# FelipeMartins96/rsoccer-isaac-cleanrl

Hardware: AMD Instinct MI355X
Metric: env-steps/s (num_envs×horizon) at 65 536 envs; PPO wall-clock to 1e8 steps (higher is better)
Workload: dtype f32; 1 GPU; vss_step FULL contract: 65536 fields/GPU, one launch per control step, random actions (BASELINE configs[1]/[2] shape); fields_per_gpu=65536, mode=full, agent_rows_per_field=1, launch=eager ctypes launches, parallelism=fields sharded over 1 GPU(s), no data-path collective

## Files before the change

### include/vss.h

```cpp
#ifndef VSS_AMD_VSS_H
#define VSS_AMD_VSS_H

#include <stdint.h>

#ifdef __cplusplus
extern "C" {
#endif

#define VSS_ABI_VERSION 2

#define VSS_NUM_TEAMS 2
#define VSS_NUM_ROBOTS 3
#define VSS_NUM_AGENTS 6
#define VSS_NUM_OBS 52
#define VSS_NUM_ACTIONS 2
#define VSS_NUM_REW 4

#define VSS_CH_BALL_X 0
#define VSS_CH_BALL_Y 1
#define VSS_CH_BALL_VX 2
#define VSS_CH_BALL_VY 3
#define VSS_CH_RX 4
#define VSS_CH_RY 10
#define VSS_CH_RQX 16
#define VSS_CH_RQY 22
#define VSS_CH_RQZ 28
#define VSS_CH_RQW 34
#define VSS_CH_RVX 40
#define VSS_CH_RVY 46
#define VSS_CH_RW 52
#define VSS_STATE_CHANNELS 58

#define VSS_MODE_FULL 0
#define VSS_MODE_SA 1
#define VSS_MODE_CMA 2
#define VSS_MODE_DMA 3


#define VSS_OK 0
#define VSS_E_ARG 1
#define VSS_E_LAUNCH 2

typedef struct vss_params {
  float w_goal;
  float w_grad;
  float w_move;
  float w_energy;
  float clip_actions;
  int32_t max_episode_length;
  uint64_t seed;
} vss_params;

typedef struct vss_state {
  float* state;
  int64_t* progress_buf;
  int64_t* reset_buf;
  float* dof_velocity_buf;
  uint32_t* rng_counter;
} vss_state;

typedef struct vss_step_io {
  const float* actions;
  float* ou_buf;
  float* obs;
  float* terminal_obs;
  float* rew;
  float* reward_sum;
  int64_t* dones_rep;
  uint8_t* time_outs;
  float* progress_f;
} vss_step_io;

typedef struct vss_rollout_io {
  const float* actions;
  float* obs;
  float* terminal_obs;
  float* rew;
  int64_t* dones;
  uint8_t* time_outs;
  float* progress_f;
} vss_rollout_io;

typedef struct vss_replay_draws {
  const float* uniforms;
  int64_t uniform_stride;
  const float* normals;
} vss_replay_draws;

int vss_abi_version(void);

const char* vss_source_hash(void);

const char* vss_error_string(int code);

int vss_step(void* stream, int64_t n_fields, int32_t mode, const vss_params* params,
             const vss_state* st, const vss_step_io* io);

int vss_step_replay(void* stream, int64_t n_fields, int32_t mode, const vss_params* params,
                    const vss_state* st, const vss_step_io* io, const vss_replay_draws* draws);

typedef struct vss_versus_io {
  const float* opp_actions;
  float* opp_obs;
} vss_versus_io;

int vss_step_versus(void* stream, int64_t n_fields, int32_t mode, const vss_params* params,
                    const vss_state* st, const vss_step_io* io, const vss_versus_io* vs);

int vss_rollout(void* stream, int64_t n_fields, int32_t n_steps, const vss_params* params,
                const vss_state* st, const vss_rollout_io* io);

int vss_reset_dones(void* stream, int64_t n_fields, const vss_params* params,
                    const vss_state* st);

int vss_reset_dones_replay(void* stream, int64_t n_fields, const vss_params* params,
                           const vss_state* st, const vss_replay_draws* draws);

int vss_compute_observations(void* stream, int64_t n_fields, const vss_state* st,
                             float* obs, int32_t n_agents);


int64_t vss_mlp_packed_size(int32_t n_out);

int vss_mlp_pack(void* stream, int32_t n_out, const float* const* weights, const float* const* biases,
                 float* packed);

int vss_policy_forward(void* stream, int64_t rows, int32_t n_act, const float* obs,
                       const float* actor_packed, const float* logstd, const float* critic_packed,
                       uint64_t seed, uint64_t counter, const float* action_in, float* action_out,
                       float* logprob_out, float* entropy_out, float* value_out, float* mean_out);

int vss_value_forward_masked(void* stream, int64_t rows, int32_t n_act, const float* obs,
                             const float* actor_packed, const float* logstd, const float* critic_packed,
                             uint64_t seed, uint64_t counter, const float* action_in, float* action_out,
                             float* logprob_out, float* entropy_out, float* value_out, float* mean_out,
                             const int64_t* row_mask);

int vss_actor_forward(void* stream, int64_t rows, int32_t n_act, const float* obs, const float* actor_packed,
                      const float* logstd, uint64_t seed, uint64_t counter, float* action_out, float* mean_out);

int vss_policy_sample(void* stream, int64_t rows, int32_t n_act, const float* mean, const float* logstd, uint64_t seed,
                      uint64_t counter, const float* action_in, float* action_out, float* logprob_out,
                      float* entropy_out);

#define VSS_MAX_ACTOR_GROUPS 16
typedef struct vss_actor_groups {
  int32_t count;
  int64_t group_rows;
  const float* actor_packed[VSS_MAX_ACTOR_GROUPS];
  const float* logstd[VSS_MAX_ACTOR_GROUPS];
} vss_actor_groups;

int vss_actor_forward_grouped(void* stream, int64_t rows, int32_t n_act, const float* obs, const vss_actor_groups* g,
                              uint64_t seed, uint64_t counter, float* action_out, float* mean_out);

int vss_policy_sample_grouped(void* stream, int64_t rows, int32_t n_act, const float* mean, const vss_actor_groups* g,
                              uint64_t seed, uint64_t counter, float* action_out);

int64_t vss_tanh_grad_chunks(int64_t rows, int32_t cols);
int vss_tanh_grad_bias(void* stream, int64_t rows, int32_t cols, const float* grad_out, const float* y,
                       float* grad_in, float* bias_partial);

int vss_linear_tanh(void* stream, int64_t rows, int32_t k_in, int32_t n_out, const float* x, const float* w,
                    const float* bias, float* y);

int vss_linear_tanh_out(void* stream, int64_t rows, int32_t k_in, int32_t n_out, const float* x, const float* w,
                        const float* bias, float* y, int32_t k_out, const float* w_out, float* out_part);

int64_t vss_linear_tanh_backward_chunks(int64_t rows, int32_t k_next, int32_t n_out);
int vss_linear_tanh_backward(void* stream, int64_t rows, int32_t k_next, int32_t n_out, const float* grad_next,
                             const float* w_next_t, const float* y, float* grad_in, float* bias_partial);

int64_t vss_output_backward_chunks(int64_t rows, int32_t k_pad, int32_t n);
int vss_output_backward(void* stream, int64_t rows, int32_t k_pad, int32_t n, const float* g_out, const float* w_out_t,
                        const float* y, float* grad_in, float* bias_partial, float* wgrad_partial);

int64_t vss_output_backward_direct_chunks(int64_t rows, int32_t k_out, int32_t n);
int vss_output_backward_direct(void* stream, int64_t rows, int32_t k_out, int32_t n, const float* g_out,
                               const float* w_out, const float* y, float* grad_in, float* bias_partial,
                               float* wgrad_partial);

int vss_linear_tanh_bf16x6(void* stream, int64_t rows, int32_t k_in, int32_t n_out, const float* x, const float* w,
                           const float* bias, float* y, uint16_t* w_split);
int vss_linear_tanh_out_bf16x6(void* stream, int64_t rows, int32_t k_in, int32_t n_out, const float* x,
                               const float* w, const float* bias, float* y, int32_t k_out, const float* w_out,
                               float* out_part, uint16_t* w_split);
int64_t vss_linear_tanh_backward_chunks_bf16x6(int64_t rows, int32_t k_next, int32_t n_out);
int vss_linear_tanh_backward_bf16x6(void* stream, int64_t rows, int32_t k_next, int32_t n_out, const float* grad_next,
                                    const float* w_next_t, const float* y, float* grad_in, float* bias_partial,
                                    uint16_t* w_split);
int64_t vss_linear_tanh_loss_blocks_bf16x6(int64_t rows, int32_t k_in, int32_t n_out);
int vss_linear_tanh_loss_bf16x6(void* stream, int32_t role, int64_t rows_pad, int64_t rows, int32_t k_in, int32_t n_out,
                                const float* x, const float* bias, int32_t k_out, const float* w_out, const float* b_out,
                                const float* action, const float* logprob_old, const float* adv, const double* adv_part,
                                int32_t adv_nparts, double adv_count, const float* logstd, const float* returns,
                                const float* values_old, float clip_coef, float clip_lo, float clip_hi, float vf_coef,
                                int32_t clip_vloss, float* grad_in, float* part_cs, float* part_dwo, float* part_stats,
                                const uint16_t* w_split);
int vss_weight_planes_bf16x6(void* stream, int32_t count, const float* const* w, const int32_t* n, const int32_t* k,
                             const int32_t* transpose, uint16_t* const* w_split);
int64_t vss_weight_grad_chunks_bf16x6(int64_t rows, int32_t n_out, int32_t k_in);
int vss_weight_grad_bf16x6(void* stream, int64_t rows, int32_t n_out, int32_t k_in, const float* grad, const float* x,
                           float* partial);
int vss_first_layer_bf16x6(void* stream, int64_t rows, int32_t k_in, int32_t n_out, const float* x, const float* w,
                           const float* bias, float* y);
int64_t vss_first_weight_grad_chunks_bf16x6(int64_t rows, int32_t n_out, int32_t k_in);
int vss_first_weight_grad_bf16x6(void* stream, int64_t rows, int32_t n_out, int32_t k_in, const float* grad,
                                 const float* x, float* partial);

int64_t vss_ppo_loss_scratch_floats(int64_t rows_pad, int32_t n_act);
int vss_ppo_loss(void* stream, int64_t rows, int64_t rows_pad, int32_t n_act, const float* mean, const float* logstd,
                 const float* value, const float* action, const float* logprob_old, const float* adv,
                 const float* returns, const float* values_old, float clip_coef, float clip_lo, float clip_hi,
                 float ent_coef, float vf_coef, int32_t clip_vloss, float* grad_mean, float* grad_value,
                 float* grad_logstd, float* loss_out, float* stats_out, float* partial);

int64_t vss_ppo_loss_direct_scratch_floats(int64_t rows_pad, int32_t n_act);
int vss_ppo_loss_direct(void* stream, int64_t rows, int64_t rows_pad, int32_t n_act, const float* mean_parts,
                        int32_t mean_nparts, const float* mean_bias, const float* value_parts, int32_t value_nparts,
                        const float* value_bias, const float* logstd, const float* action, const float* logprob_old,
                        const float* adv, const double* adv_part, int32_t adv_nparts, double adv_count,
                        const float* returns, const float* values_old, float clip_coef, float clip_lo, float clip_hi,
                        float ent_coef, float vf_coef, int32_t clip_vloss, float* grad_mean, float* grad_value,
                        float* grad_logstd, float* grad_mean_bias, float* grad_value_bias, float* loss_out,
                        float* stats_out, float* partial);
int vss_ppo_loss_fused_finish(void* stream, int64_t rows, int32_t n_act, int64_t actor_blocks, const float* actor_stats,
                              int64_t critic_blocks, const float* critic_stats, const float* logstd, float ent_coef,
                              float vf_coef, float* grad_logstd, float* grad_mean_bias, float* grad_value_bias,
                              float* loss_out, float* stats_out);
int64_t vss_randperm_scratch_bytes(int64_t n);
int vss_randperm(void* stream, int64_t n, const int64_t* seed, int64_t* out, void* scratch, int64_t scratch_bytes);
int vss_randperm_bits(void* stream, int64_t n, int32_t key_bits, const int64_t* seed, int64_t* out, void* scratch,
                      int64_t scratch_bytes);
int64_t vss_minibatch_gather_parts(int64_t mb);
int vss_minibatch_gather(void* stream, int64_t mb, int64_t rows_pad, int64_t batch, const int64_t* inds, int64_t obs_w,
                         int64_t act_w, const float* b_obs, const float* b_act, const float* b_logp, const float* b_adv,
                         const float* b_ret, const float* b_val, float* obs, float* act, float* logp, float* adv,
                         float* ret, float* val, double* adv_part);
int vss_adv_part_sum(void* stream, int32_t nparts, const double* part, double* out);

int64_t vss_grad_sq_partials_count(int64_t n);
int vss_grad_sq_partials(void* stream, int64_t n, const float* grad, float* partial);
int vss_adam_step_clipped(void* stream, int64_t n, int32_t nparts, const float* partial, float max_norm, float lr,
                          float beta1, float beta2, float eps, int64_t step, float* grad, float* param, float* exp_avg,
                          float* exp_avg_sq, float* norm_out);
int vss_sum_parts(void* stream, int32_t count, const float* const* src, float* const* dst, const int64_t* parts,
                  const int64_t* part_stride, const int64_t* rows, const int64_t* cols, const int64_t* src_ld,
                  const int64_t* dst_ld);

int vss_episode_stats(void* stream, int64_t rows, const float* rews, const int64_t* dones, float* ep_returns,
                      int32_t* ep_lengths, float* returned_returns, int32_t* returned_lengths, float* return_sum);

int vss_match_tally(void* stream, int64_t n_fields, int32_t rows_per_field, int64_t group_fields, int32_t count,
                    const float* rew, const int64_t* dones, const float* progress_f, int64_t* tally);

#ifdef __cplusplus
}
#endif

#endif
```

### rsoccer-isaac-cleanrl_amd/csrc/vss_gemm_x6.hip

```cpp
#include <hip/hip_runtime.h>
#include <stdint.h>

#include <type_traits>

#include "../../include/vss.h"
#include "vss_loss_row.h"

#if defined(__HIP_DEVICE_COMPILE__) && !defined(__gfx950__)
#error "vss_gemm_x6.hip targets gfx950 (CDNA4) only: v_mfma_f32_16x16x32_bf16, v_cvt_pk_bf16_f32"
#endif


namespace vx6 {

typedef __bf16 bf16x8 __attribute__((ext_vector_type(8)));
typedef __bf16 bf16x2 __attribute__((ext_vector_type(2)));
typedef float f32x4 __attribute__((ext_vector_type(4)));
typedef uint32_t u32x4 __attribute__((ext_vector_type(4)));

typedef short i16x4 __attribute__((ext_vector_type(4)));

enum { EPI_TANH = 0, EPI_DTANH = 1, EPI_TANH_OUT = 2, EPI_WGRAD = 3, EPI_LOSS_A = 4, EPI_LOSS_C = 5 };
enum { ST_ROW = 0, ST_TR = 1, ST_DMA = 2, ST_TR2 = 3, ST_KROW = 4 };

constexpr int KT = 32;
constexpr int kYPre = 1;

__device__ __forceinline__ float tanh_f32(float z) {
  const float a = fabsf(z), s = z * z;
  const float poly = z + z * s * (-0.333333343f + s * (0.133333340f + s * (-0.0539682545f + s * 0.0218694885f)));
  const float t = __builtin_amdgcn_exp2f(-2.8853900817779268f * a);
  const float ex = copysignf((1.0f - t) * __builtin_amdgcn_rcpf(1.0f + t), z);
  return a < 0.3f ? poly : ex;
}

__device__ __forceinline__ uint32_t pk_bf16(float a, float b) {
  const bf16x2 v = {(__bf16)a, (__bf16)b};
  return __builtin_bit_cast(uint32_t, v);
}

__device__ __forceinline__ void split8(const float (&v)[8], u32x4& hi, u32x4& mid, u32x4& lo) {
#pragma unroll
  for (int p = 0; p < 4; ++p) {
    const float a = v[2 * p], b = v[2 * p + 1];
    const uint32_t h = pk_bf16(a, b);
    const float ra = a - __uint_as_float(h << 16), rb = b - __uint_as_float(h & 0xFFFF0000u);
    const uint32_t m = pk_bf16(ra, rb);
    const float sa = ra - __uint_as_float(m << 16), sb = rb - __uint_as_float(m & 0xFFFF0000u);
    const uint32_t l = __builtin_amdgcn_perm(__float_as_uint(sb), __float_as_uint(sa), 0x07060302u);
    hi[p] = h;
    mid[p] = m;
    lo[p] = l;
  }
}

template <int R>
struct Img {
  static constexpr int GS = R * 16;
  static constexpr int PS = 4 * GS;
  static constexpr int BYTES = 3 * PS;
};

__device__ __forceinline__ int kswz(int r) { return ((r & 3) << 2) | ((r >> 2) & 3); }
template <int R>
struct KImg {
  static constexpr int SUB = 32 * 256;
  static constexpr int PS = (R / 128) * SUB;
  static_assert(R % 128 == 0 && 3 * PS == Img<R>::BYTES, "ST_KROW: whole 128-feature sub-tiles, same bytes as Img");
};
__device__ __forceinline__ int kfrag_off(int i0, int lane, int h) {
  const int q = (lane >> 2) & 3, p = lane & 3, row = 8 * (lane >> 4) + 4 * h + q;
  const int c = ((i0 & 127) >> 3) + (p >> 1);
  return (i0 >> 7) * (32 * 256) + row * 256 + 16 * (c ^ kswz(row)) + 8 * (p & 1);
}
__device__ __forceinline__ u32x4 tr_frag(const char* lds_at_a, const char* lds_at_b) {
  typedef __attribute__((address_space(3))) i16x4* lp;
  const i16x4 a = __builtin_amdgcn_ds_read_tr16_b64_v4i16((lp)(lds_at_a));
  const i16x4 b = __builtin_amdgcn_ds_read_tr16_b64_v4i16((lp)(lds_at_b));
  const uint2 ua = __builtin_bit_cast(uint2, a), ub = __builtin_bit_cast(uint2, b);
  return (u32x4){ua.x, ua.y, ub.x, ub.y};
}

template <int BI_, int BJ_, int WI_, int WJ_>
struct Cfg {
  static constexpr int BI = BI_, BJ = BJ_, WI = WI_, WJ = WJ_;
  static constexpr int THREADS = 64 * WI * WJ;
  static constexpr int WTI = BI / WI, WTJ = BJ / WJ;
  static constexpr int TI = WTI / 16, TJ = WTJ / 16;
  static constexpr int PI = BI * 4 / THREADS, PJ = BJ * 4 / THREADS;
  static constexpr int BUF = Img<BI>::BYTES + Img<BJ>::BYTES;
  static constexpr int LDS = 2 * BUF;
  static_assert(PI * THREADS == BI * 4 && PJ * THREADS == BJ * 4, "staging pairs must tile the block");
  static_assert(WTI == 64, "a wave's i extent is one 64-feature slice (EPI_TANH_OUT)");
  static constexpr int BPC = 2 * LDS <= 160 * 1024 ? 2 : 1;
  static_assert(LDS <= 160 * 1024, "the LDS image must fit a CU");
};
using CfgA = Cfg<128, 256, 2, 4>;
using CfgB = Cfg<256, 128, 4, 2>;

struct Args {
  int32_t ni, nj;
  int64_t kpairs;
  int32_t items;
  int32_t splits;
  int64_t ldp, ldq;
  const void* p;
  const float* q;
  int64_t ldo;
  float* out;
  const float* bias;
  const float* y;
  float* partial;
  const float* w_out;
  float* out_part;
  const float* b_out;
  const float* l_act;
  const float* l_logp;
  const float* l_adv;
  const double* adv_part;
  int32_t adv_nparts;
  double adv_count;
  const float* logstd;
  const float* l_ret;
  const float* l_val;
  float clip, clip_lo, clip_hi, vf_coef, inv_n;
  int32_t clip_vloss;
  int64_t rows_real;
  float* part_cs;
  float* part_dwo;
  float* part_stats;
};

constexpr int kLossStats = vlossrow::kBlockStats;

template <int NP>
struct Stage {
  u32x4 v[NP][2];
};

template <int MODE, int R, int NP, class C>
__device__ __forceinline__ void load_op(u32x4 (*dst)[2], const void* base_, int64_t ld, int64_t k0) {
  const int t = threadIdx.x;
  if constexpr (MODE == ST_TR2) {
    static_assert(NP == 2 && (R / 2) * 4 == C::THREADS, "ST_TR2: one column pair x 4 k groups per thread");
    const int c2 = t % (R / 2), g = t / (R / 2);
    const float* src = static_cast<const float*>(base_) + (k0 + 8 * g) * ld + 2 * c2;
#pragma unroll
    for (int e = 0; e < 8; ++e) {
      const float2 x = *reinterpret_cast<const float2*>(src + e * ld);
      dst[0][e >> 2][e & 3] = __float_as_uint(x.x);
      dst[1][e >> 2][e & 3] = __float_as_uint(x.y);
    }
    return;
  }
#pragma unroll
  for (int u = 0; u < NP; ++u) {
    const int pr = t + C::THREADS * u;
    if constexpr (MODE == ST_KROW) {
      const int row = pr / (R / 8), cc = pr % (R / 8);
      const float* src = static_cast<const float*>(base_) + (k0 + row) * ld + 8 * cc;
      dst[u][0] = *reinterpret_cast<const u32x4*>(src);
      dst[u][1] = *reinterpret_cast<const u32x4*>(src + 4);
    } else if constexpr (MODE == ST_ROW) {
      const int g = (pr >> 3) & 3, row = (pr & 7) | ((pr >> 5) << 3);
      const float* src = static_cast<const float*>(base_) + (int64_t)row * ld + k0 + 8 * g;
      dst[u][0] = *reinterpret_cast<const u32x4*>(src);
      dst[u][1] = *reinterpret_cast<const u32x4*>(src + 4);
    } else {
      const int row = pr % R, g = pr / R;
      const float* src = static_cast<const float*>(base_) + (k0 + 8 * g) * ld + row;
#pragma unroll
      for (int e = 0; e < 8; ++e) dst[u][e >> 2][e & 3] = __float_as_uint(src[e * ld]);
    }
  }
}

template <int MODE, int R, int NP, class C>
__device__ __forceinline__ void write_op(const u32x4 (*src)[2], char* img) {
  const int t = threadIdx.x;
#pragma unroll
  for (int u = 0; u < NP; ++u) {
    const int pr = t + C::THREADS * u;
    int g, row;
    if constexpr (MODE == ST_TR) {
      row = pr % R;
      g = pr / R;
    } else if constexpr (MODE == ST_TR2) {
      row = 2 * (t % (R / 2)) + u;
      g = t / (R / 2);
    } else {
      g = (pr >> 3) & 3;
      row = (pr & 7) | ((pr >> 5) << 3);
    }
    u32x4 hi, mid, lo;
    float v[8];
#pragma unroll
    for (int e = 0; e < 8; ++e) v[e] = __uint_as_float(src[u][e >> 2][e & 3]);
    split8(v, hi, mid, lo);
    char* d;
    int ps;
    if constexpr (MODE == ST_KROW) {
      const int kr = pr / (R / 8), cc = pr % (R / 8);
      d = img + (cc >> 4) * KImg<R>::SUB + kr * 256 + 16 * ((cc & 15) ^ kswz(kr));
      ps = KImg<R>::PS;
    } else {
      d = img + g * Img<R>::GS + row * 16;
      ps = Img<R>::PS;
    }
    *reinterpret_cast<u32x4*>(d) = hi;
    *reinterpret_cast<u32x4*>(d + ps) = mid;
    *reinterpret_cast<u32x4*>(d + 2 * ps) = lo;
  }
}

template <int R>
__global__ __launch_bounds__(256) void split_image_kernel(const float* __restrict__ w, int64_t n, int64_t k,
                                                          uint16_t* __restrict__ img) {
  const int64_t ktn = k / KT, units = n * k / 8;
  const int64_t u = (int64_t)blockIdx.x * 256 + threadIdx.x;
  if (u >= units) return;
  const int r = (int)(u % R), g = (int)((u / R) % 4);
  const int64_t kt = (u / (4 * R)) % ktn, it = u / (4 * R * ktn);
  const float* src = w + (it * R + r) * k + kt * KT + 8 * g;
  const u32x4 a = *reinterpret_cast<const u32x4*>(src), b = *reinterpret_cast<const u32x4*>(src + 4);
  float v[8];
#pragma unroll
  for (int e = 0; e < 4; ++e) {
    v[e] = __uint_as_float(a[e]);
    v[4 + e] = __uint_as_float(b[e]);
  }
  u32x4 hi, mid, lo;
  split8(v, hi, mid, lo);
  uint16_t* d = img + (it * ktn + kt) * (3 * 4 * R * 8) + (g * R + r) * 8;
  *reinterpret_cast<u32x4*>(d) = hi;
  *reinterpret_cast<u32x4*>(d + 4 * R * 8) = mid;
  *reinterpret_cast<u32x4*>(d + 2 * 4 * R * 8) = lo;
}

struct PlaneJob {
  const float* w;
  uint16_t* img;
  int64_t n, k;
  int32_t trans, r;
};
constexpr int kMaxPlaneJobs = 16;
struct PlaneJobs {
  PlaneJob j[kMaxPlaneJobs];
};

__global__ __launch_bounds__(256) void plane_images_kernel(PlaneJobs jobs) {
  const PlaneJob& J = jobs.j[blockIdx.y];
  const int64_t ktn = J.k / KT, units = J.n * J.k / 8;
  const int64_t u = (int64_t)blockIdx.x * 256 + threadIdx.x;
  if (u >= units) return;
  const int R = J.r;
  const int r = (int)(u % R), g = (int)((u / R) % 4);
  const int64_t kt = (u / (4 * R)) % ktn, it = u / (4 * R * ktn);
  const int64_t row = it * R + r, col = kt * KT + 8 * g;
  float v[8];
  if (J.trans) {
#pragma unroll
    for (int e = 0; e < 8; ++e) v[e] = J.w[(col + e) * J.n + row];
  } else {
    const u32x4 a = *reinterpret_cast<const u32x4*>(J.w + row * J.k + col);
    const u32x4 b = *reinterpret_cast<const u32x4*>(J.w + row * J.k + col + 4);
#pragma unroll
    for (int e = 0; e < 4; ++e) {
      v[e] = __uint_as_float(a[e]);
      v[4 + e] = __uint_as_float(b[e]);
    }
  }
  u32x4 hi, mid, lo;
  split8(v, hi, mid, lo);
  uint16_t* d = J.img + (it * ktn + kt) * (3 * 4 * (int64_t)R * 8) + ((int64_t)g * R + r) * 8;
  *reinterpret_cast<u32x4*>(d) = hi;
  *reinterpret_cast<u32x4*>(d + 4 * R * 8) = mid;
  *reinterpret_cast<u32x4*>(d + 2 * 4 * R * 8) = lo;
}

template <int CTRL>
__device__ __forceinline__ float dpp_f32(float x) {
  return __int_as_float(__builtin_amdgcn_update_dpp(0, __float_as_int(x), CTRL, 0xF, 0xF, false));
}
__device__ __forceinline__ float row16_sum(float v) {
  v += dpp_f32<0xB1>(v);
  v += dpp_f32<0x4E>(v);
  v += dpp_f32<0x141>(v);
  v += dpp_f32<0x140>(v);
  return v;
}
__device__ __forceinline__ float kgroup_sum(float v) {
  const auto a = __builtin_amdgcn_permlane16_swap(__float_as_uint(v), __float_as_uint(v), false, false);
  v = __uint_as_float(a[0]) + __uint_as_float(a[1]);
  const auto b = __builtin_amdgcn_permlane32_swap(__float_as_uint(v), __float_as_uint(v), false, false);
  return __uint_as_float(b[0]) + __uint_as_float(b[1]);
}
__device__ __forceinline__ float wave64_sum(float v) { return kgroup_sum(row16_sum(v)); }
__device__ __forceinline__ float lane_sel(uint64_t m, float a, float b) {
  float r;
  asm("v_cndmask_b32_e64 %0, %1, %2, %3" : "=v"(r) : "v"(a), "v"(b), "s"(m));
  return r;
}
__device__ __forceinline__ float pick16(const float (&t)[16], int k) {
  const uint64_t m0 = __builtin_amdgcn_ballot_w64(k & 1), m1 = __builtin_amdgcn_ballot_w64(k & 2),
                 m2 = __builtin_amdgcn_ballot_w64(k & 4), m3 = __builtin_amdgcn_ballot_w64(k & 8);
  float a[8], b[4], c[2];
#pragma unroll
  for (int m = 0; m < 8; ++m) a[m] = lane_sel(m0, t[2 * m], t[2 * m + 1]);
#pragma unroll
  for (int m = 0; m < 4; ++m) b[m] = lane_sel(m1, a[2 * m], a[2 * m + 1]);
#pragma unroll
  for (int m = 0; m < 2; ++m) c[m] = lane_sel(m2, b[2 * m], b[2 * m + 1]);
  return lane_sel(m3, c[0], c[1]);
}

template <int EPI, int SP, int SQ, class C, int KO = 0>
__global__ __launch_bounds__(C::THREADS, C::BPC) void gemm_x6_kernel(Args a) {
  constexpr int BI = C::BI, BJ = C::BJ, TI = C::TI, TJ = C::TJ, PJ = C::PJ;
  constexpr bool PDMA = SP == ST_DMA;
  constexpr int PI = PDMA ? 0 : C::PI;
  constexpr int NQ = Img<BI>::BYTES / (C::THREADS / 64) / 1024;
  static_assert(!PDMA || NQ * (C::THREADS / 64) * 1024 == Img<BI>::BYTES, "DMA slices: whole KB per wave");
  constexpr bool LOSS = EPI == EPI_LOSS_A || EPI == EPI_LOSS_C;
  constexpr int E_P = BI + KO * 256, E_CS = E_P + C::WI * BJ * KO, E_DW = E_CS + C::WJ * BI,
                E_ST = E_DW + C::WJ * KO * BI, E_AD = E_ST + 2 * kLossStats;
  constexpr int EPI_FLOATS = LOSS ? E_AD + 2
                                  : (EPI == EPI_TANH_OUT ? KO * 256 + BI
                                                         : (EPI == EPI_WGRAD ? 1 : (EPI == EPI_DTANH ? C::WJ * BI : BI)));
  static_assert(!LOSS || (BI == 256 && KO >= 1 && KO <= 2), "EPI_LOSS_*: whole 256-feature rows, 1 or 2 outputs");
  __shared__ __attribute__((aligned(16))) char lds[C::LDS + EPI_FLOATS * 4];
  float* epi_lds = reinterpret_cast<float*>(lds + C::LDS);
  const int tid = threadIdx.x, lane = tid & 63, wv = tid >> 6, wi = wv / C::WJ, wj = wv % C::WJ;
  const int G = gridDim.x;
  const int slot = (G % 8 == 0) ? (int)(blockIdx.x % 8) * (G / 8) + (int)(blockIdx.x / 8) : (int)blockIdx.x;
  if (slot >= a.items) return;
  const int per_split = a.ni * a.nj;

  auto item_ij = [&](int w, int& it, int& jt, int& sp) {
    sp = w / per_split;
    const int r = w % per_split;
    jt = r / a.ni;
    it = r % a.ni;
  };

  int it0, jt0, sp0;
  item_ij(slot, it0, jt0, sp0);
  if constexpr (EPI != EPI_WGRAD) {
    for (int i = tid; i < (EPI == EPI_DTANH ? EPI_FLOATS : BI); i += C::THREADS)
      epi_lds[i] = EPI == EPI_DTANH ? 0.f : a.bias[it0 * BI + i];
    if constexpr (EPI == EPI_TANH_OUT || LOSS)
      for (int i = tid; i < KO * 256; i += C::THREADS) epi_lds[BI + i] = a.w_out[i];
    if constexpr (LOSS) {
      for (int i = E_CS + tid; i < E_AD; i += C::THREADS) epi_lds[i] = 0.f;
      if (EPI == EPI_LOSS_A && a.adv_part && wv == 0) {
        double s0 = 0.0, q0 = 0.0;
        for (int i = lane; i < a.adv_nparts; i += 64) {
          s0 += a.adv_part[2 * i];
          q0 += a.adv_part[2 * i + 1];
        }
#pragma unroll
        for (int m = 32; m >= 1; m >>= 1) {
          s0 += __shfl_xor(s0, m);
          q0 += __shfl_xor(q0, m);
        }
        if (lane == 0) {
          const double n = a.adv_count, m = s0 / n;
          double var = (q0 - n * m * m) / (n - 1.0);
          var = var > 0.0 ? var : 0.0;
          epi_lds[E_AD] = (float)m;
          epi_lds[E_AD + 1] = (float)sqrt(var);
        }
      }
    }
  }

  int f_item = slot, f_kt = 0;
  const char* fp;
  const char* fq;
  auto kt_lo = [&](int sp) -> int64_t {
    if constexpr (EPI == EPI_WGRAD) return 2 * ((int64_t)sp * a.kpairs / a.splits);
    return sp == 0 ? 0 : 2 * a.kpairs;
  };
  int64_t fk0 = 0;
  int f_kn = 0;
  auto point = [&](int w) {
    int it, jt, sp;
    item_ij(w, it, jt, sp);
    fk0 = kt_lo(sp) * KT;
    f_kn = (int)(kt_lo(sp + 1) - kt_lo(sp));
    if constexpr (SP == ST_TR || SP == ST_KROW) fp = static_cast<const char*>(a.p) + (int64_t)it * BI * 4;
    else fp = static_cast<const char*>(a.p);
    if constexpr (SQ == ST_TR || SQ == ST_TR2 || SQ == ST_KROW)
      fq = reinterpret_cast<const char*>(a.q) + (int64_t)jt * BJ * 4;
    else fq = reinterpret_cast<const char*>(a.q) + (int64_t)jt * BJ * a.ldq * 4;
  };
  point(f_item);
  auto gload = [&](Stage<PI + PJ>& s) {
    const int64_t k0 = fk0 + (int64_t)f_kt * KT;
    if constexpr (!PDMA) load_op<SP, BI, PI, C>(s.v, fp, a.ldp, k0);
    load_op<SQ, BJ, PJ, C>(s.v + PI, fq, a.ldq, k0);
    if (++f_kt >= f_kn) {
      if (f_item + G < a.items) {
        f_kt = 0;
        f_item += G;
        point(f_item);
      } else {
        f_kt = f_kn - 1;
      }
    }
  };
  auto swrite = [&](const Stage<PI + PJ>& s, int buf) {
    char* base = lds + buf * C::BUF;
    if constexpr (!PDMA) write_op<SP, BI, PI, C>(s.v, base);
    write_op<SQ, BJ, PJ, C>(s.v + PI, base + Img<BI>::BYTES);
  };
  auto dma_p = [&](int64_t kt, int buf) {
    if constexpr (PDMA) {
      const int64_t off = ((int64_t)it0 * (2 * a.kpairs) + kt) * Img<BI>::BYTES;
#pragma unroll
      for (int q = 0; q < NQ; ++q) {
        const int slice = (wv * NQ + q) * 1024;
        __builtin_amdgcn_global_load_lds(
            (__attribute__((address_space(1))) void*)(static_cast<const char*>(a.p) + off + slice + lane * 16),
            (__attribute__((address_space(3))) void*)(lds + buf * C::BUF + slice), 16, 0, 0);
      }
    }
  };

  f32x4 acc[TI][TJ];
  const int fr = lane & 15, fg = lane >> 4;
  auto mfma_tile = [&](int buf, auto&& between) {
    const char* pb = lds + buf * C::BUF + fg * Img<BI>::GS + (wi * C::WTI + fr) * 16;
    const char* qb = lds + buf * C::BUF + Img<BI>::BYTES + fg * Img<BJ>::GS + (wj * C::WTJ + fr) * 16;
    u32x4 pf[3][TI], qf[3][TJ];
    const char* pk = lds + buf * C::BUF;
    const char* qk = lds + buf * C::BUF + Img<BI>::BYTES;
#pragma unroll
    for (int pl = 0; pl < 3; ++pl) {
#pragma unroll
      for (int i = 0; i < TI; ++i) {
        if constexpr (SP == ST_KROW) {
          const int i0 = wi * C::WTI + 16 * i;
          pf[pl][i] = tr_frag(pk + pl * KImg<BI>::PS + kfrag_off(i0, lane, 0), pk + pl * KImg<BI>::PS + kfrag_off(i0, lane, 1));
        } else {
          pf[pl][i] = *reinterpret_cast<const u32x4*>(pb + pl * Img<BI>::PS + i * 256);
        }
      }
#pragma unroll
      for (int j = 0; j < TJ; ++j) {
        if constexpr (SQ == ST_KROW) {
          const int j0 = wj * C::WTJ + 16 * j;
          qf[pl][j] = tr_frag(qk + pl * KImg<BJ>::PS + kfrag_off(j0, lane, 0), qk + pl * KImg<BJ>::PS + kfrag_off(j0, lane, 1));
        } else {
          qf[pl][j] = *reinterpret_cast<const u32x4*>(qb + pl * Img<BJ>::PS + j * 256);
        }
      }
    }
    if constexpr (PDMA) {
      __builtin_amdgcn_sched_barrier(0);
      between();
      __builtin_amdgcn_sched_barrier(0);
    }
    constexpr int PP[6] = {2, 0, 1, 1, 0, 0};
    constexpr int QP[6] = {0, 2, 1, 0, 1, 0};
#pragma unroll
    for (int x = 0; x < 6; ++x)
#pragma unroll
      for (int i = 0; i < TI; ++i)
#pragma unroll
        for (int j = 0; j < TJ; ++j)
          acc[i][j] = __builtin_amdgcn_mfma_f32_16x16x32_bf16(__builtin_bit_cast(bf16x8, pf[PP[x]][i]),
                                                              __builtin_bit_cast(bf16x8, qf[QP[x]][j]), acc[i][j], 0, 0, 0);
  };

  auto loss_epilogue = [&](f32x4 (&ac)[TI][TJ], int it, int jt) __attribute__((always_inline)) {
    if constexpr (LOSS) {
      const int ib = it * BI + wi * C::WTI;
      const int64_t grow = (int64_t)jt * BJ + tid;
      const bool row_real = tid < BJ && grow < a.rows_real;
      float in_x[KO], in_b[KO], in_ls[KO], in_a = 0.f, in_l = 0.f;
#pragma unroll
      for (int o = 0; o < KO; ++o) in_x[o] = in_b[o] = in_ls[o] = 0.f;
      if (tid < BJ) {
#pragma unroll
        for (int o = 0; o < KO; ++o) {
          in_b[o] = a.b_out[o];
          if constexpr (EPI == EPI_LOSS_A) in_ls[o] = a.logstd[o];
        }
        if (row_real) {
          if constexpr (EPI == EPI_LOSS_A) {
#pragma unroll
            for (int o = 0; o < KO; ++o) in_x[o] = a.l_act[grow * KO + o];
            in_a = a.l_adv[grow];
            in_l = a.l_logp[grow];
          } else {
            in_a = a.l_ret[grow];
            in_l = a.clip_vloss ? a.l_val[grow] : 0.f;
          }
        }
      }
#pragma unroll
      for (int j = 0; j < TJ; ++j) {
        const int rl = wj * C::WTJ + 16 * j + fr;
        float od[KO];
#pragma unroll
        for (int o = 0; o < KO; ++o) od[o] = 0.f;
#pragma unroll
        for (int i = 0; i < TI; ++i) {
          const int il = wi * C::WTI + 16 * i + 4 * fg;
          f32x4 v = ac[i][j];
#pragma unroll
          for (int r = 0; r < 4; ++r) v[r] = tanh_f32(v[r] + epi_lds[il + r]);
          ac[i][j] = v;
#pragma unroll
          for (int o = 0; o < KO; ++o) {
            const float* wo = epi_lds + BI + o * 256 + ib + 16 * i + 4 * fg;
            float d = v[0] * wo[0];
            d = fmaf(v[1], wo[1], d);
            d = fmaf(v[2], wo[2], d);
            d = fmaf(v[3], wo[3], d);
            od[o] += d;
          }
        }
#pragma unroll
        for (int o = 0; o < KO; ++o) {
          const float d = kgroup_sum(od[o]);
          if (fg == 0) epi_lds[E_P + (wi * BJ + rl) * KO + o] = d;
        }
      }
      __syncthreads();
      if (tid < BJ) {
        float outv[KO], g[KO], t[kLossStats > 0 ? 5 + 2 * KO : 1];
#pragma unroll
        for (int o = 0; o < KO; ++o) {
          float d = epi_lds[E_P + tid * KO + o];
#pragma unroll
          for (int q = 1; q < C::WI; ++q) d += epi_lds[E_P + (q * BJ + tid) * KO + o];
          outv[o] = d + in_b[o];
          g[o] = 0.f;
        }
#pragma unroll
        for (int k = 0; k < 5 + 2 * KO; ++k) t[k] = 0.f;
        if (row_real) {
          if constexpr (EPI == EPI_LOSS_A) {
            float var[KO], lsc[KO], gm[KO], lg[KO];
            vlossrow::actor_consts<KO>(in_ls, var, lsc);
            float A = in_a;
            if (a.adv_part) A = (A - epi_lds[E_AD]) / (epi_lds[E_AD + 1] + 1e-8f);
            vlossrow::actor_row<KO>(outv, in_x, in_l, A, var, lsc, a.clip, a.clip_lo, a.clip_hi, a.inv_n, t[0], t[2],
                                    t[3], t[4], gm, lg);
#pragma unroll
            for (int o = 0; o < KO; ++o) {
              g[o] = gm[o];
              t[5 + o] = lg[o];
              t[5 + KO + o] = gm[o];
            }
          } else {
            float gv;
            vlossrow::critic_row(outv[0], in_a, in_l, a.clip_vloss, a.clip, a.vf_coef, a.inv_n, t[1], gv);
            g[0] = gv;
            t[5] = gv;
          }
        }
#pragma unroll
        for (int o = 0; o < KO; ++o) epi_lds[E_P + tid * KO + o] = g[o];
        float ts[16];
#pragma unroll
        for (int k = 0; k < 16; ++k) ts[k] = k < 5 + 2 * KO ? wave64_sum(t[k]) : 0.f;
        const float tv = pick16(ts, fr);
        if (lane < 5 + 2 * KO) epi_lds[E_ST + wv * kLossStats + lane] += tv;
      }
      __syncthreads();
#pragma unroll
      for (int i = 0; i < TI; ++i) {
        const int il = wi * C::WTI + 16 * i + 4 * fg;
        float cs[4] = {0.f, 0.f, 0.f, 0.f}, dw[4][KO];
#pragma unroll
        for (int r = 0; r < 4; ++r)
#pragma unroll
          for (int o = 0; o < KO; ++o) dw[r][o] = 0.f;
#pragma unroll
        for (int j = 0; j < TJ; ++j) {
          const int rl = wj * C::WTJ + 16 * j + fr;
          const int64_t jg = (int64_t)jt * BJ + rl;
          float g[KO];
#pragma unroll
          for (int o = 0; o < KO; ++o) g[o] = epi_lds[E_P + rl * KO + o];
          const f32x4 v = ac[i][j];
          vx6::f32x4 z;
#pragma unroll
          for (int r = 0; r < 4; ++r) {
            float sg = g[0] * epi_lds[BI + il + r];
#pragma unroll
            for (int o = 1; o < KO; ++o) sg = fmaf(g[o], epi_lds[BI + o * 256 + il + r], sg);
            z[r] = sg * fmaf(-v[r], v[r], 1.0f);
            cs[r] += z[r];
#pragma unroll
            for (int o = 0; o < KO; ++o) dw[r][o] = fmaf(g[o], v[r], dw[r][o]);
          }
          __builtin_nontemporal_store(z, reinterpret_cast<f32x4*>(a.out + jg * a.ldo + ib + 16 * i + 4 * fg));
        }
        float t[16];
#pragma unroll
        for (int r = 0; r < 4; ++r) {
          t[r] = row16_sum(cs[r]);
#pragma unroll
          for (int o = 0; o < KO; ++o) t[4 + 4 * o + r] = row16_sum(dw[r][o]);
        }
#pragma unroll
        for (int k = 4 + 4 * KO; k < 16; ++k) t[k] = 0.f;
        const float v = pick16(t, fr);
        if (fr < 4 + 4 * KO) {
          const int slot = fr < 4 ? E_CS + wj * BI + il + fr : E_DW + (wj * KO + ((fr - 4) >> 2)) * BI + il + (fr & 3);
          epi_lds[slot] += v;
        }
      }
    }
  };

  Stage<PI + PJ> r0, r1;
  gload(r0);
  dma_p(0, 0);
  swrite(r0, 0);
  gload(r1);
  gload(r0);
  __syncthreads();
  int w = slot;
  for (;;) {
    const int next = w + G;
    const bool has_next = next < a.items;
    int it, jt, sp;
    item_ij(w, it, jt, sp);
#pragma unroll
    for (int i = 0; i < TI; ++i)
#pragma unroll
      for (int j = 0; j < TJ; ++j) acc[i][j] = (f32x4){0.f, 0.f, 0.f, 0.f};
    f32x4 ypre[EPI == EPI_DTANH ? kYPre : 1][EPI == EPI_DTANH ? TI : 1];
    const int64_t jy = (int64_t)jt * BJ + wj * C::WTJ + fr;
    const int kn = (int)(kt_lo(sp + 1) - kt_lo(sp));
    for (int kt = 0; kt < kn; kt += 2) {
      if constexpr (EPI == EPI_DTANH) {
        if (kt + 2 >= kn) {
#pragma unroll
          for (int j = 0; j < kYPre; ++j)
#pragma unroll
            for (int i = 0; i < TI; ++i)
              ypre[j][i] = *reinterpret_cast<const f32x4*>(a.y + (jy + 16 * j) * a.ldo + it * BI + wi * C::WTI + 16 * i +
                                                           4 * fg);
        }
      }
      mfma_tile(0, [&] { dma_p(kt + 1, 1); });
      swrite(r1, 1);
      __syncthreads();
      gload(r1);
      mfma_tile(1, [&] {
        if (kt + 2 < kn) dma_p(kt + 2, 0);
        else if (has_next) dma_p(0, 0);
      });
      swrite(r0, 0);
      __syncthreads();
      gload(r0);
    }

    float cs[EPI == EPI_DTANH ? TI : 1][4];
#pragma unroll
    for (int i = 0; i < (EPI == EPI_DTANH ? TI : 1); ++i) cs[i][0] = cs[i][1] = cs[i][2] = cs[i][3] = 0.f;
    const int ib = it * BI + wi * C::WTI, jb = jt * BJ + wj * C::WTJ;
    if constexpr (LOSS) {
      loss_epilogue(acc, it, jt);
      if (!has_next) break;
      w = next;
      continue;
    }
    f32x4 yrest[EPI == EPI_DTANH ? TJ : 1][EPI == EPI_DTANH ? TI : 1];
    if constexpr (EPI == EPI_DTANH) {
#pragma unroll
      for (int j = kYPre; j < TJ; ++j)
#pragma unroll
        for (int i = 0; i < TI; ++i)
          yrest[j][i] = *reinterpret_cast<const f32x4*>(a.y + ((int64_t)jb + 16 * j + fr) * a.ldo + ib + 16 * i + 4 * fg);
    }
#pragma unroll
    for (int j = 0; j < TJ; ++j) {
      const int64_t jg = (int64_t)jb + 16 * j + fr;
      float od[KO > 0 ? KO : 1];
#pragma unroll
      for (int o = 0; o < (KO > 0 ? KO : 1); ++o) od[o] = 0.f;
#pragma unroll
      for (int i = 0; i < TI; ++i) {
        const int il = wi * C::WTI + 16 * i + 4 * fg;
        const int ig = it * BI + il;
        f32x4 v = acc[i][j];
        if constexpr (EPI == EPI_TANH || EPI == EPI_TANH_OUT) {
#pragma unroll
          for (int r = 0; r < 4; ++r) v[r] = tanh_f32(v[r] + epi_lds[il + r]);
          *reinterpret_cast<f32x4*>(a.out + jg * a.ldo + ig) = v;
          if constexpr (EPI == EPI_TANH_OUT) {
#pragma unroll
            for (int o = 0; o < KO; ++o) {
              const float* wo = epi_lds + BI + o * 256 + ig;
              float d = v[0] * wo[0];
              d = fmaf(v[1], wo[1], d);
              d = fmaf(v[2], wo[2], d);
              d = fmaf(v[3], wo[3], d);
              od[o] += d;
            }
          }
        } else if constexpr (EPI == EPI_DTANH) {
          const f32x4 yv = j < kYPre ? ypre[j < kYPre ? j : 0][i] : yrest[j][i];
#pragma unroll
          for (int r = 0; r < 4; ++r) {
            v[r] = v[r] * fmaf(-yv[r], yv[r], 1.0f);
            cs[i][r] += v[r];
          }
          acc[i][j] = v;
        } else {
          *reinterpret_cast<f32x4*>(a.out + ((int64_t)sp * a.nj * BJ + jg) * a.ldo + ig) = v;
        }
      }
      if constexpr (EPI == EPI_DTANH) {
#pragma unroll
        for (int i = 0; i < TI; i += 2) {
          f32x4 lo8, hi8;
#pragma unroll
          for (int r = 0; r < 4; ++r) {
            const float xr = dpp_f32<0x128>(acc[i][j][r]), yr = dpp_f32<0x128>(acc[i + 1][j][r]);
            lo8[r] = fr < 8 ? acc[i][j][r] : yr;
            hi8[r] = fr < 8 ? xr : acc[i + 1][j][r];
          }
          const int64_t r0 = (int64_t)jb + 16 * j + (fr & 7);
          const int64_t col = (int64_t)it * BI + wi * C::WTI + 16 * (i + (fr >> 3)) + 4 * fg;
          float* d0 = a.out + r0 * a.ldo + col;
          float* d1 = a.out + (r0 + 8) * a.ldo + col;
          if constexpr (EPI == EPI_DTANH) {
            __builtin_nontemporal_store(lo8, reinterpret_cast<f32x4*>(d0));
            __builtin_nontemporal_store(hi8, reinterpret_cast<f32x4*>(d1));
          } else {
            *reinterpret_cast<f32x4*>(d0) = lo8;
            *reinterpret_cast<f32x4*>(d1) = hi8;
          }
        }
      }
      if constexpr (EPI == EPI_TANH_OUT) {
#pragma unroll
        for (int o = 0; o < KO; ++o) {
          const float d = kgroup_sum(od[o]);
          if (fg == 0) a.out_part[(((int64_t)ib >> 6) * (a.nj * BJ) + jg) * KO + o] = d;
        }
      }
    }
    if constexpr (EPI == EPI_DTANH) {
      static_assert(EPI != EPI_DTANH || TI == 4, "EPI_DTANH column sums: 4 feature tiles per wave");
      float t[16];
#pragma unroll
      for (int i = 0; i < TI; ++i)
#pragma unroll
        for (int r = 0; r < 4; ++r) t[4 * i + r] = row16_sum(cs[i][r]);
      epi_lds[wj * BI + wi * C::WTI + 16 * (fr >> 2) + 4 * fg + (fr & 3)] += pick16(t, fr);
    }
    if (!has_next) break;
    w = next;
  }

  if constexpr (LOSS) {
    __syncthreads();
    for (int f = tid; f < BI; f += C::THREADS) {
      float t = epi_lds[E_CS + f];
#pragma unroll
      for (int m = 1; m < C::WJ; ++m) t += epi_lds[E_CS + m * BI + f];
      a.part_cs[(int64_t)slot * BI + f] = t;
    }
    for (int x = tid; x < KO * BI; x += C::THREADS) {
      const int o = x / BI, f = x - o * BI;
      float t = epi_lds[E_DW + o * BI + f];
#pragma unroll
      for (int m = 1; m < C::WJ; ++m) t += epi_lds[E_DW + (m * KO + o) * BI + f];
      a.part_dwo[((int64_t)slot * KO + o) * BI + f] = t;
    }
    if (tid < kLossStats) a.part_stats[(int64_t)slot * kLossStats + tid] = epi_lds[E_ST + tid] + epi_lds[E_ST + kLossStats + tid];
  }
  if constexpr (EPI == EPI_DTANH) {
    __syncthreads();
    for (int f = tid; f < BI; f += C::THREADS) {
      float t = epi_lds[f];
#pragma unroll
      for (int m = 1; m < C::WJ; ++m) t += epi_lds[m * BI + f];
      a.partial[(int64_t)(slot / a.ni) * (a.ni * BI) + it0 * BI + f] = t;
    }
  }
}

constexpr int FW_THREADS = 512, FW_N = 256, FW_KMAX = 64;
constexpr int FW_XPS = 16 * 256;
constexpr int FW_GPS = KImg<FW_N>::PS;
constexpr int FW_BUF = 3 * FW_GPS + 3 * FW_XPS;
constexpr int FW_NX = (32 * FW_KMAX / 4 + FW_THREADS - 1) / FW_THREADS;
constexpr int FW_NG = 32 * FW_N / 8 / FW_THREADS;

__device__ __forceinline__ int fw_xoff(int r, int c) {
  const int rho = r & 15, phi = c + 64 * (r >> 4);
  return rho * 256 + 16 * ((phi >> 3) ^ kswz(rho)) + 8 * ((phi >> 2) & 1);
}

__global__ __launch_bounds__(FW_THREADS, 1) void first_wgrad_kernel(int64_t kpairs, int32_t k_in, const float* __restrict__ grad,
                                                                      const float* __restrict__ x, float* __restrict__ partial) {
  __shared__ __attribute__((aligned(16))) char lds[2 * FW_BUF];
  const int tid = threadIdx.x, lane = tid & 63, wv = tid >> 6;
  const int G = gridDim.x, b = blockIdx.x;
  const int64_t kt0 = 2 * ((int64_t)b * kpairs / G), kn = 2 * (((int64_t)b + 1) * kpairs / G) - kt0;
  const int xchunks = 8 * k_in;
  for (int i = tid; i < 2 * 3 * FW_XPS / 16; i += FW_THREADS) {
    const int buf = i / (3 * FW_XPS / 16), o = i % (3 * FW_XPS / 16);
    *reinterpret_cast<u32x4*>(lds + buf * FW_BUF + 3 * FW_GPS + 16 * o) = (u32x4){0u, 0u, 0u, 0u};
  }
  struct St {
    u32x4 g[FW_NG][2];
    u32x4 x[FW_NX];
  };
  int64_t f_kt = 0;
  auto gload = [&](St& s) {
    const int64_t kt = kt0 + (f_kt < kn ? f_kt : kn - 1);
    ++f_kt;
    const float* gsrc = grad + kt * 32 * FW_N;
#pragma unroll
    for (int u = 0; u < FW_NG; ++u) {
      const int pr = tid + FW_THREADS * u, row = pr >> 5, cc = pr & 31;
      s.g[u][0] = *reinterpret_cast<const u32x4*>(gsrc + row * FW_N + 8 * cc);
      s.g[u][1] = *reinterpret_cast<const u32x4*>(gsrc + row * FW_N + 8 * cc + 4);
    }
    const float* xsrc = x + kt * 32 * k_in;
#pragma unroll
    for (int u = 0; u < FW_NX; ++u) {
      const int ch = tid + FW_THREADS * u;
      if (ch < xchunks) s.x[u] = *reinterpret_cast<const u32x4*>(xsrc + 4 * ch);
    }
  };
  auto swrite = [&](const St& s, int buf) {
    char* gimg = lds + buf * FW_BUF;
#pragma unroll
    for (int u = 0; u < FW_NG; ++u) {
      const int pr = tid + FW_THREADS * u, row = pr >> 5, cc = pr & 31;
      float v[8];
#pragma unroll
      for (int e = 0; e < 8; ++e) v[e] = __uint_as_float(s.g[u][e >> 2][e & 3]);
      u32x4 hi, mid, lo;
      split8(v, hi, mid, lo);
      char* d = gimg + (cc >> 4) * KImg<FW_N>::SUB + row * 256 + 16 * ((cc & 15) ^ kswz(row));
      *reinterpret_cast<u32x4*>(d) = hi;
      *reinterpret_cast<u32x4*>(d + FW_GPS) = mid;
      *reinterpret_cast<u32x4*>(d + 2 * FW_GPS) = lo;
    }
    char* ximg = lds + buf * FW_BUF + 3 * FW_GPS;
    const int cpr = k_in >> 2;
#pragma unroll
    for (int u = 0; u < FW_NX; ++u) {
      const int ch = tid + FW_THREADS * u;
      if (ch < xchunks) {
        float v[8];
#pragma unroll
        for (int e = 0; e < 4; ++e) {
          v[e] = __uint_as_float(s.x[u][e]);
          v[4 + e] = 0.f;
        }
        u32x4 hi, mid, lo;
        split8(v, hi, mid, lo);
        char* d = ximg + fw_xoff(ch / cpr, 4 * (ch % cpr));
        *reinterpret_cast<uint2*>(d) = (uint2){hi[0], hi[1]};
        *reinterpret_cast<uint2*>(d + FW_XPS) = (uint2){mid[0], mid[1]};
        *reinterpret_cast<uint2*>(d + 2 * FW_XPS) = (uint2){lo[0], lo[1]};
      }
    }
  };
  const int fs = wv & 3, cs = wv >> 2;
  f32x4 acc[4][2];
#pragma unroll
  for (int i = 0; i < 4; ++i)
#pragma unroll
    for (int j = 0; j < 2; ++j) acc[i][j] = (f32x4){0.f, 0.f, 0.f, 0.f};
  const int q = (lane >> 2) & 3, p = lane & 3, fg = lane >> 4;
  auto mfma_tile = [&](int buf) {
    const char* gk = lds + buf * FW_BUF;
    const char* xk = lds + buf * FW_BUF + 3 * FW_GPS;
    u32x4 pf[3][4], qf[3][2];
#pragma unroll
    for (int pl = 0; pl < 3; ++pl) {
#pragma unroll
      for (int i = 0; i < 4; ++i) {
        const int i0 = 64 * fs + 16 * i;
        pf[pl][i] = tr_frag(gk + pl * FW_GPS + kfrag_off(i0, lane, 0), gk + pl * FW_GPS + kfrag_off(i0, lane, 1));
      }
#pragma unroll
      for (int j = 0; j < 2; ++j) {
        const int r0 = 8 * fg + q, c0 = 16 * (2 * cs + j) + 4 * p;
        qf[pl][j] = tr_frag(xk + pl * FW_XPS + fw_xoff(r0, c0), xk + pl * FW_XPS + fw_xoff(r0 + 4, c0));
      }
    }
    constexpr int PP[6] = {2, 0, 1, 1, 0, 0};
    constexpr int QP[6] = {0, 2, 1, 0, 1, 0};
#pragma unroll
    for (int xx = 0; xx < 6; ++xx)
#pragma unroll
      for (int i = 0; i < 4; ++i)
#pragma unroll
        for (int j = 0; j < 2; ++j)
          acc[i][j] = __builtin_amdgcn_mfma_f32_16x16x32_bf16(__builtin_bit_cast(bf16x8, pf[PP[xx]][i]),
                                                              __builtin_bit_cast(bf16x8, qf[QP[xx]][j]), acc[i][j], 0, 0, 0);
  };
  St r0, r1;
  __syncthreads();
  gload(r0);
  swrite(r0, 0);
  gload(r1);
  gload(r0);
  __syncthreads();
  for (int64_t kt = 0; kt < kn; kt += 2) {
    mfma_tile(0);
    swrite(r1, 1);
    __syncthreads();
    gload(r1);
    mfma_tile(1);
    swrite(r0, 0);
    __syncthreads();
    gload(r0);
  }
  const int fr = lane & 15;
#pragma unroll
  for (int j = 0; j < 2; ++j) {
    const int c = 16 * (2 * cs + j) + fr;
    if (c < k_in) {
#pragma unroll
      for (int i = 0; i < 4; ++i)
#pragma unroll
        for (int r = 0; r < 4; ++r) partial[((int64_t)b * FW_N + 64 * fs + 16 * i + 4 * fg + r) * k_in + c] = acc[i][j][r];
    }
  }
}

static int fw_parts(int64_t rows) {
  const int64_t pairs = rows / (2 * KT);
  int64_t g = pairs / 8;
  if (g > 256) g = 256;
  if (g < 1) g = 1;
  return (int)g;
}

constexpr int kGridCus = 256;

struct Plan {
  int32_t ni, nj, splits, items, grid;
  int64_t kpairs;
};

template <class C>
static bool fb_shape_ok(int64_t rows, int32_t k, int32_t n) {
  return rows > 0 && rows % C::BJ == 0 && rows / C::BJ <= (1 << 22) && n > 0 && n % C::BI == 0 && n <= 4096 &&
         k > 0 && k % (2 * KT) == 0 && k <= 65536 && (rows / C::BJ) * (n / C::BI) <= 0x3fffffff;
}

template <class C>
static Plan fb_plan(int64_t rows, int32_t k, int32_t n) {
  Plan p;
  p.ni = n / C::BI;
  p.nj = (int32_t)(rows / C::BJ);
  p.kpairs = k / (2 * KT);
  p.splits = 1;
  p.items = p.ni * p.nj;
  int g = kGridCus * C::BPC;
  g -= g % (8 * p.ni);
  p.grid = (g > 0 && g < p.items) ? g : p.items;
  return p;
}

template <class F>
static auto with_fb_cfg(int32_t n, F&& f) {
  return n > 0 && n % CfgB::BI == 0 ? f(CfgB{}) : f(CfgA{});
}

static bool wg_shape_ok(int64_t rows, int32_t n_out, int32_t k_in) {
  return rows > 0 && rows % (2 * KT) == 0 && rows <= (int64_t(1) << 36) && k_in > 0 && k_in % CfgA::BI == 0 &&
         k_in <= 4096 && n_out > 0 && n_out % CfgA::BJ == 0 && n_out <= 4096;
}

static Plan wg_plan(int64_t rows, int32_t n_out, int32_t k_in) {
  Plan p;
  p.ni = k_in / CfgA::BI;
  p.nj = n_out / CfgA::BJ;
  const int64_t pairs = rows / (2 * KT);
  const int tiles = p.ni * p.nj;
  int64_t s = kGridCus * CfgA::BPC / tiles;
  if (s < 1) s = 1;
  if (s > pairs) s = pairs;
  p.splits = (int32_t)s;
  p.kpairs = pairs;
  p.items = tiles * s;
  p.grid = p.items < kGridCus * CfgA::BPC ? p.items : kGridCus * CfgA::BPC;
  p.grid -= (p.grid % 8 && p.grid > 8) ? p.grid % 8 : 0;
  return p;
}

template <int EPI, int SP, int SQ, class C, int KO = 0>
static int launch(void* stream, Args a, const Plan& pl) {
  a.ni = pl.ni;
  a.nj = pl.nj;
  a.kpairs = pl.kpairs;
  a.items = pl.items;
  a.splits = pl.splits;
  hipLaunchKernelGGL((gemm_x6_kernel<EPI, SP, SQ, C, KO>), dim3((unsigned)pl.grid), dim3(C::THREADS), 0,
                     (hipStream_t)stream, a);
  return hipGetLastError() == hipSuccess ? VSS_OK : VSS_E_LAUNCH;
}

static bool misaligned(const void* p) { return !p || (reinterpret_cast<uintptr_t>(p) & 15) != 0; }

template <class C>
static int split_weight(void* stream, const float* w, int64_t n, int64_t k, uint16_t* w_split) {
  const int64_t units = n * k / 8;
  hipLaunchKernelGGL(split_image_kernel<C::BI>, dim3((unsigned)((units + 255) / 256)), dim3(256), 0,
                     (hipStream_t)stream, w, n, k, w_split);
  return hipGetLastError() == hipSuccess ? VSS_OK : VSS_E_LAUNCH;
}

static Args fb_args(int32_t k, int32_t n, const uint16_t* w_split, const float* q, float* out) {
  Args a{};
  a.ldp = k;
  a.ldq = k;
  a.p = w_split;
  a.q = q;
  a.ldo = n;
  a.out = out;
  return a;
}

constexpr int FL_WAVES = 8, FL_THREADS = 64 * FL_WAVES;
__global__ __launch_bounds__(FL_THREADS) void first_layer_x6_kernel(int64_t rows, int k, const float* __restrict__ x,
                                                                    const float* __restrict__ w,
                                                                    const float* __restrict__ bias,
                                                                    float* __restrict__ y) {
  __shared__ u32x4 wimg[2 * 3 * 16 * 64];
  __shared__ float bl[256];
  for (int p = threadIdx.x; p < 256 * 8; p += FL_THREADS) {
    const int f = p >> 3, g = p & 7;
    float v[8];
#pragma unroll
    for (int e = 0; e < 8; ++e) {
      const int kk = 8 * g + e;
      v[e] = kk < k ? w[(int64_t)f * k + kk] : 0.0f;
    }
    u32x4 pl[3];
    split8(v, pl[0], pl[1], pl[2]);
    const int ks = g >> 2, fg = g & 3, it = f >> 4, fr = f & 15;
#pragma unroll
    for (int q = 0; q < 3; ++q) wimg[((ks * 3 + q) * 16 + it) * 64 + fg * 16 + fr] = pl[q];
  }
  for (int i = threadIdx.x; i < 256; i += FL_THREADS) bl[i] = bias[i];
  __syncthreads();
  const int lane = threadIdx.x & 63, wv = threadIdx.x >> 6, fr = lane & 15, fg = lane >> 4;
  const int64_t slabs = (rows + 15) / 16, step = (int64_t)gridDim.x * FL_WAVES;
  auto load_x = [&](int64_t sl, float4 (&xr)[2][2]) __attribute__((always_inline)) {
    const int64_t row = sl * 16 + fr;
#pragma unroll
    for (int ks = 0; ks < 2; ++ks)
#pragma unroll
      for (int h = 0; h < 2; ++h) {
        const int k0 = 32 * ks + 8 * fg + 4 * h;
        xr[ks][h] = (row < rows && k0 + 4 <= k) ? *reinterpret_cast<const float4*>(x + row * k + k0)
                                                 : make_float4(0.f, 0.f, 0.f, 0.f);
      }
  };
  constexpr int PP[6] = {2, 0, 1, 1, 0, 0};
  constexpr int QP[6] = {0, 2, 1, 0, 1, 0};
  int64_t sl = (int64_t)blockIdx.x * FL_WAVES + wv;
  float4 xr[2][2];
  if (sl < slabs) load_x(sl, xr);
  for (; sl < slabs; sl += step) {
    u32x4 xp[2][3];
#pragma unroll
    for (int ks = 0; ks < 2; ++ks) {
      const float v[8] = {xr[ks][0].x, xr[ks][0].y, xr[ks][0].z, xr[ks][0].w,
                          xr[ks][1].x, xr[ks][1].y, xr[ks][1].z, xr[ks][1].w};
      split8(v, xp[ks][0], xp[ks][1], xp[ks][2]);
    }
    if (sl + step < slabs) load_x(sl + step, xr);
    f32x4 acc[16];
#pragma unroll
    for (int i = 0; i < 16; ++i) acc[i] = (f32x4){0.f, 0.f, 0.f, 0.f};
#pragma unroll
    for (int st = 0; st < 8; ++st) {
      const int ig = st >> 1, ks = st & 1;
      u32x4 pf[3][4];
#pragma unroll
      for (int q = 0; q < 3; ++q)
#pragma unroll
        for (int ii = 0; ii < 4; ++ii) pf[q][ii] = wimg[((ks * 3 + q) * 16 + 4 * ig + ii) * 64 + lane];
#pragma unroll
      for (int xx = 0; xx < 6; ++xx)
#pragma unroll
        for (int ii = 0; ii < 4; ++ii)
          acc[4 * ig + ii] = __builtin_amdgcn_mfma_f32_16x16x32_bf16(__builtin_bit_cast(bf16x8, pf[PP[xx]][ii]),
                                                                     __builtin_bit_cast(bf16x8, xp[ks][QP[xx]]),
                                                                     acc[4 * ig + ii], 0, 0, 0);
      __builtin_amdgcn_sched_barrier(0);
    }
    const int64_t row = sl * 16 + fr;
    if (row < rows) {
#pragma unroll
      for (int i = 0; i < 16; ++i) {
        const int f0 = 16 * i + 4 * fg;
        f32x4 v = acc[i];
#pragma unroll
        for (int r = 0; r < 4; ++r) v[r] = tanh_f32(v[r] + bl[f0 + r]);
        *reinterpret_cast<f32x4*>(y + row * 256 + f0) = v;
      }
    }
  }
}

}

extern "C" {

int vss_linear_tanh_bf16x6(void* stream, int64_t rows, int32_t k_in, int32_t n_out, const float* x, const float* w,
                           const float* bias, float* y, uint16_t* w_split) {
  using namespace vx6;
  return with_fb_cfg(n_out, [&](auto cfg) {
    using C = decltype(cfg);
    if (!fb_shape_ok<C>(rows, k_in, n_out) || (w && misaligned(w)) || misaligned(x) || misaligned(y) || !bias ||
        misaligned(w_split))
      return (int)VSS_E_ARG;
    int rc = w ? split_weight<C>(stream, w, n_out, k_in, w_split) : VSS_OK;
    if (rc != VSS_OK) return rc;
    Args a = fb_args(k_in, n_out, w_split, x, y);
    a.bias = bias;
    return launch<EPI_TANH, ST_DMA, ST_ROW, C>(stream, a, fb_plan<C>(rows, k_in, n_out));
  });
}

int vss_linear_tanh_out_bf16x6(void* stream, int64_t rows, int32_t k_in, int32_t n_out, const float* x, const float* w,
                               const float* bias, float* y, int32_t k_out, const float* w_out, float* out_part,
                               uint16_t* w_split) {
  using namespace vx6;
  return with_fb_cfg(n_out, [&](auto cfg) {
    using C = decltype(cfg);
    if (!fb_shape_ok<C>(rows, k_in, n_out) || n_out != 256 || misaligned(x) || (w && misaligned(w)) || misaligned(y) ||
        !bias || !w_out || !out_part || !(k_out == 1 || k_out == 2 || k_out == 6) || misaligned(w_split))
      return (int)VSS_E_ARG;
    int rc = w ? split_weight<C>(stream, w, n_out, k_in, w_split) : VSS_OK;
    if (rc != VSS_OK) return rc;
    Args a = fb_args(k_in, n_out, w_split, x, y);
    a.bias = bias;
    a.w_out = w_out;
    a.out_part = out_part;
    const Plan pl = fb_plan<C>(rows, k_in, n_out);
    if (k_out == 1) return launch<EPI_TANH_OUT, ST_DMA, ST_ROW, C, 1>(stream, a, pl);
    if (k_out == 2) return launch<EPI_TANH_OUT, ST_DMA, ST_ROW, C, 2>(stream, a, pl);
    return launch<EPI_TANH_OUT, ST_DMA, ST_ROW, C, 6>(stream, a, pl);
  });
}

int64_t vss_linear_tanh_loss_blocks_bf16x6(int64_t rows, int32_t k_in, int32_t n_out) {
  using namespace vx6;
  if (n_out != 256 || !fb_shape_ok<CfgB>(rows, k_in, n_out)) return -1;
  return fb_plan<CfgB>(rows, k_in, n_out).grid;
}

int vss_linear_tanh_loss_bf16x6(void* stream, int32_t role, int64_t rows_pad, int64_t rows, int32_t k_in, int32_t n_out,
                                const float* x, const float* bias, int32_t k_out, const float* w_out, const float* b_out,
                                const float* action, const float* logprob_old, const float* adv, const double* adv_part,
                                int32_t adv_nparts, double adv_count, const float* logstd, const float* returns,
                                const float* values_old, float clip_coef, float clip_lo, float clip_hi, float vf_coef,
                                int32_t clip_vloss, float* grad_in, float* part_cs, float* part_dwo, float* part_stats,
                                const uint16_t* w_split) {
  using namespace vx6;
  using C = CfgB;
  const bool actor = role == 0;
  if ((role != 0 && role != 1) || n_out != 256 || !fb_shape_ok<C>(rows_pad, k_in, n_out) || rows <= 0 || rows > rows_pad ||
      misaligned(x) || misaligned(grad_in) || misaligned(w_split) || !bias || !w_out || !b_out || !part_cs || !part_dwo ||
      !part_stats || (actor && (k_out < 1 || k_out > 2 || !action || !logprob_old || !adv || !logstd ||
                                (adv_part && (adv_nparts < 1 || !(adv_count > 1.0))))) ||
      (!actor && (k_out != 1 || !returns || (clip_vloss && !values_old))))
    return VSS_E_ARG;
  Args a = fb_args(k_in, n_out, w_split, x, grad_in);
  a.bias = bias;
  a.w_out = w_out;
  a.b_out = b_out;
  a.l_act = action;
  a.l_logp = logprob_old;
  a.l_adv = adv;
  a.adv_part = adv_part;
  a.adv_nparts = adv_nparts;
  a.adv_count = adv_count;
  a.logstd = logstd;
  a.l_ret = returns;
  a.l_val = values_old;
  a.clip = clip_coef;
  a.clip_lo = clip_lo;
  a.clip_hi = clip_hi;
  a.vf_coef = vf_coef;
  a.inv_n = 1.0f / (float)rows;
  a.clip_vloss = clip_vloss;
  a.rows_real = rows;
  a.part_cs = part_cs;
  a.part_dwo = part_dwo;
  a.part_stats = part_stats;
  const Plan pl = fb_plan<C>(rows_pad, k_in, n_out);
  if (!actor) return launch<EPI_LOSS_C, ST_DMA, ST_ROW, C, 1>(stream, a, pl);
  if (k_out == 1) return launch<EPI_LOSS_A, ST_DMA, ST_ROW, C, 1>(stream, a, pl);
  return launch<EPI_LOSS_A, ST_DMA, ST_ROW, C, 2>(stream, a, pl);
}

int64_t vss_linear_tanh_backward_chunks_bf16x6(int64_t rows, int32_t k_next, int32_t n_out) {
  using namespace vx6;
  return with_fb_cfg(n_out, [&](auto cfg) -> int64_t {
    using C = decltype(cfg);
    if (!fb_shape_ok<C>(rows, k_next, n_out)) return -1;
    const Plan pl = fb_plan<C>(rows, k_next, n_out);
    return pl.grid / pl.ni;
  });
}

int vss_linear_tanh_backward_bf16x6(void* stream, int64_t rows, int32_t k_next, int32_t n_out, const float* grad_next,
                                    const float* w_next_t, const float* y, float* grad_in, float* bias_partial,
                                    uint16_t* w_split) {
  using namespace vx6;
  return with_fb_cfg(n_out, [&](auto cfg) {
    using C = decltype(cfg);
    if (!fb_shape_ok<C>(rows, k_next, n_out) || misaligned(grad_next) || (w_next_t && misaligned(w_next_t)) ||
        misaligned(y) || misaligned(grad_in) || misaligned(bias_partial) || misaligned(w_split))
      return (int)VSS_E_ARG;
    int rc = w_next_t ? split_weight<C>(stream, w_next_t, n_out, k_next, w_split) : VSS_OK;
    if (rc != VSS_OK) return rc;
    Args a = fb_args(k_next, n_out, w_split, grad_next, grad_in);
    a.y = y;
    a.partial = bias_partial;
    return launch<EPI_DTANH, ST_DMA, ST_ROW, C>(stream, a, fb_plan<C>(rows, k_next, n_out));
  });
}

int vss_weight_planes_bf16x6(void* stream, int32_t count, const float* const* w, const int32_t* n, const int32_t* k,
                             const int32_t* transpose, uint16_t* const* w_split) {
  using namespace vx6;
  if (count < 1 || count > kMaxPlaneJobs || !w || !n || !k || !transpose || !w_split) return VSS_E_ARG;
  PlaneJobs jobs{};
  int64_t blocks = 0;
  for (int q = 0; q < count; ++q) {
    const int32_t nq = n[q], kq = k[q];
    if (nq <= 0 || nq % CfgA::BI || nq > 4096 || kq <= 0 || kq % (2 * KT) || kq > 65536 || !w[q] ||
        misaligned(w_split[q]) || (transpose[q] != 0 && transpose[q] != 1) ||
        (!transpose[q] && misaligned(w[q])))
      return VSS_E_ARG;
    jobs.j[q] = PlaneJob{w[q], w_split[q], nq, kq, transpose[q], nq % CfgB::BI == 0 ? CfgB::BI : CfgA::BI};
    const int64_t b = ((int64_t)nq * kq / 8 + 255) / 256;
    if (b > blocks) blocks = b;
  }
  hipLaunchKernelGGL(plane_images_kernel, dim3((unsigned)blocks, (unsigned)count), dim3(256), 0, (hipStream_t)stream,
                     jobs);
  return hipGetLastError() == hipSuccess ? VSS_OK : VSS_E_LAUNCH;
}

int64_t vss_weight_grad_chunks_bf16x6(int64_t rows, int32_t n_out, int32_t k_in) {
  using namespace vx6;
  if (!wg_shape_ok(rows, n_out, k_in)) return -1;
  return wg_plan(rows, n_out, k_in).splits;
}

int vss_weight_grad_bf16x6(void* stream, int64_t rows, int32_t n_out, int32_t k_in, const float* grad, const float* x,
                           float* partial) {
  using namespace vx6;
  if (!wg_shape_ok(rows, n_out, k_in) || misaligned(grad) || misaligned(x) || misaligned(partial)) return VSS_E_ARG;
  Args a{};
  a.ldp = k_in;
  a.ldq = n_out;
  a.p = x;
  a.q = grad;
  a.ldo = k_in;
  a.out = partial;
  return launch<EPI_WGRAD, ST_KROW, ST_KROW, CfgA>(stream, a, wg_plan(rows, n_out, k_in));
}

int64_t vss_first_weight_grad_chunks_bf16x6(int64_t rows, int32_t n_out, int32_t k_in) {
  using namespace vx6;
  if (rows <= 0 || rows % (2 * KT) || rows > (int64_t(1) << 36) || n_out != FW_N || k_in <= 0 || k_in > FW_KMAX ||
      k_in % 4)
    return -1;
  return fw_parts(rows);
}

int vss_first_weight_grad_bf16x6(void* stream, int64_t rows, int32_t n_out, int32_t k_in, const float* grad,
                                 const float* x, float* partial) {
  using namespace vx6;
  if (vss_first_weight_grad_chunks_bf16x6(rows, n_out, k_in) < 0 || misaligned(grad) || misaligned(x) || !partial)
    return VSS_E_ARG;
  const int g = fw_parts(rows);
  hipLaunchKernelGGL(first_wgrad_kernel, dim3((unsigned)g), dim3(FW_THREADS), 0, (hipStream_t)stream,
                     (int64_t)(rows / (2 * KT)), k_in, grad, x, partial);
  return hipGetLastError() == hipSuccess ? VSS_OK : VSS_E_LAUNCH;
}

int vss_first_layer_bf16x6(void* stream, int64_t rows, int32_t k_in, int32_t n_out, const float* x, const float* w,
                           const float* bias, float* y) {
  using namespace vx6;
  if (rows < 0 || n_out != 256 || k_in <= 0 || k_in > 64 || k_in % 4 != 0 || misaligned(x) || !w || !bias ||
      misaligned(y))
    return VSS_E_ARG;
  if (rows == 0) return VSS_OK;
  int64_t g = ((rows + 15) / 16 + FL_WAVES - 1) / FL_WAVES;
  if (g > 256) g = 256;
  hipLaunchKernelGGL(first_layer_x6_kernel, dim3((unsigned)g), dim3(FL_THREADS), 0, (hipStream_t)stream, rows, k_in, x,
                     w, bias, y);
  return hipGetLastError() == hipSuccess ? VSS_OK : VSS_E_LAUNCH;
}

}
```

### rsoccer-isaac-cleanrl_amd/vss_amd/_native.py

```python
from __future__ import annotations

import ctypes
import hashlib
import os

import torch

HERE = os.path.dirname(os.path.abspath(__file__))
TOOLS = os.path.join(os.path.dirname(os.path.dirname(HERE)), "tools")


def _lib_path() -> str:
    alt = os.environ.get("VSS_LIB_PATH")
    if not alt:
        return os.path.join(HERE, "libvss_amd.so")
    alt = os.path.realpath(alt)
    if not alt.startswith(os.path.realpath(TOOLS) + os.sep):
        raise RuntimeError(f"VSS_LIB_PATH={alt}: only variant builds under {TOOLS} are accepted")
    import warnings
    warnings.warn(f"libvss_amd: loading the variant build {alt} (VSS_LIB_PATH)", RuntimeWarning)
    return alt


LIB_PATH = _lib_path()
CSRC = os.path.join(os.path.dirname(HERE), "csrc")
HEADER = os.path.join(os.path.dirname(os.path.dirname(HERE)), "include", "vss.h")

STAMPED = (os.path.join(CSRC, "vss_step.hip"), os.path.join(CSRC, "vss_update.hip"),
           os.path.join(CSRC, "vss_policy.hip"), os.path.join(CSRC, "vss_gemm_x6.hip"),
           os.path.join(CSRC, "vss_loss.hip"), os.path.join(CSRC, "vss_optim.hip"),
           os.path.join(CSRC, "vss_loss_row.h"), HEADER,
           os.path.join(CSRC, "Makefile"))

ABI_VERSION = 2
MODE_FULL, MODE_SA, MODE_CMA, MODE_DMA = 0, 1, 2, 3
STATE_CHANNELS = 58
CH_BALL_X, CH_BALL_Y, CH_BALL_VX, CH_BALL_VY = 0, 1, 2, 3
CH_RX, CH_RY, CH_RQX, CH_RQY, CH_RQZ, CH_RQW, CH_RVX, CH_RVY, CH_RW = 4, 10, 16, 22, 28, 34, 40, 46, 52
EXPORTED = ("vss_abi_version", "vss_source_hash", "vss_error_string", "vss_step", "vss_step_replay", "vss_step_versus",
            "vss_actor_forward", "vss_actor_forward_grouped", "vss_policy_sample_grouped", "vss_match_tally",
            "vss_rollout", "vss_reset_dones",
            "vss_reset_dones_replay",
            "vss_compute_observations", "vss_mlp_packed_size", "vss_mlp_pack", "vss_policy_forward",
            "vss_value_forward_masked", "vss_policy_sample", "vss_episode_stats", "vss_tanh_grad_chunks", "vss_tanh_grad_bias",
            "vss_linear_tanh", "vss_linear_tanh_out", "vss_linear_tanh_backward_chunks", "vss_linear_tanh_backward",
            "vss_output_backward_chunks", "vss_output_backward", "vss_linear_tanh_bf16x6",
            "vss_linear_tanh_out_bf16x6", "vss_linear_tanh_backward_chunks_bf16x6", "vss_linear_tanh_backward_bf16x6",
            "vss_weight_grad_chunks_bf16x6", "vss_weight_grad_bf16x6", "vss_first_weight_grad_chunks_bf16x6",
            "vss_first_weight_grad_bf16x6", "vss_weight_planes_bf16x6", "vss_ppo_loss_scratch_floats", "vss_ppo_loss",
            "vss_grad_sq_partials_count", "vss_grad_sq_partials", "vss_adam_step_clipped", "vss_sum_parts",
            "vss_output_backward_direct_chunks", "vss_output_backward_direct", "vss_ppo_loss_direct_scratch_floats",
            "vss_ppo_loss_direct", "vss_minibatch_gather_parts", "vss_minibatch_gather", "vss_adv_part_sum",
            "vss_first_layer_bf16x6", "vss_linear_tanh_loss_blocks_bf16x6", "vss_linear_tanh_loss_bf16x6",
            "vss_ppo_loss_fused_finish", "vss_randperm_scratch_bytes", "vss_randperm", "vss_randperm_bits")


class VssParams(ctypes.Structure):
    _fields_ = [
        ("w_goal", ctypes.c_float),
        ("w_grad", ctypes.c_float),
        ("w_move", ctypes.c_float),
        ("w_energy", ctypes.c_float),
        ("clip_actions", ctypes.c_float),
        ("max_episode_length", ctypes.c_int32),
        ("seed", ctypes.c_uint64),
    ]


class VssState(ctypes.Structure):
    _fields_ = [(k, ctypes.c_void_p) for k in
                ("state", "progress_buf", "reset_buf", "dof_velocity_buf", "rng_counter")]


class VssStepIO(ctypes.Structure):
    _fields_ = [(k, ctypes.c_void_p) for k in
                ("actions", "ou_buf", "obs", "terminal_obs", "rew", "reward_sum", "dones_rep",
                 "time_outs", "progress_f")]


class VssVersusIO(ctypes.Structure):
    _fields_ = [(k, ctypes.c_void_p) for k in ("opp_actions", "opp_obs")]


MAX_ACTOR_GROUPS = 16


class VssActorGroups(ctypes.Structure):
    _fields_ = [("count", ctypes.c_int32), ("group_rows", ctypes.c_int64),
                ("actor_packed", ctypes.c_void_p * MAX_ACTOR_GROUPS), ("logstd", ctypes.c_void_p * MAX_ACTOR_GROUPS)]


class VssRolloutIO(ctypes.Structure):
    _fields_ = [(k, ctypes.c_void_p) for k in
                ("actions", "obs", "terminal_obs", "rew", "dones", "time_outs", "progress_f")]


class VssReplayDraws(ctypes.Structure):
    _fields_ = [("uniforms", ctypes.c_void_p), ("uniform_stride", ctypes.c_int64), ("normals", ctypes.c_void_p)]


class NativeError(RuntimeError):
    pass


_lib = None


def source_hash() -> str:
    h = hashlib.sha256()
    for path in STAMPED:
        with open(path, "rb") as f:
            h.update(f.read())
    return h.hexdigest()[:16]


def verify_source_hash(lib: ctypes.CDLL, expected: str | None = None) -> None:
    want = source_hash() if expected is None else expected
    try:
        fn = lib.vss_source_hash
    except AttributeError:
        fn = None
    if fn is not None:
        fn.restype = ctypes.c_char_p
    built = fn().decode() if fn is not None else "<no vss_source_hash symbol>"
    if built != want:
        raise NativeError(
            f"{LIB_PATH} was built from other sources (stamp {built}, tree {want}); rebuild it with "
            f"`make -C {CSRC}` or `python -c 'import __graft_entry__ as g; g.build()'`")


def load() -> ctypes.CDLL:
    global _lib
    if _lib is not None:
        return _lib
    if not os.path.exists(LIB_PATH):
        raise NativeError(
            f"VSS HIP library not found at {LIB_PATH}; build it with "
            f"`make -C {CSRC}` or `python -c 'import __graft_entry__ as g; g.build()'`")
    L = ctypes.CDLL(LIB_PATH)
    verify_source_hash(L)
    P, i64, i32 = ctypes.c_void_p, ctypes.c_int64, ctypes.c_int32
    L.vss_abi_version.restype = ctypes.c_int
    L.vss_error_string.argtypes = [ctypes.c_int]
    L.vss_error_string.restype = ctypes.c_char_p
    L.vss_step.argtypes = [P, i64, i32, P, P, P]
    L.vss_step.restype = ctypes.c_int
    L.vss_step_replay.argtypes = [P, i64, i32, P, P, P, P]
    L.vss_step_replay.restype = ctypes.c_int
    L.vss_step_versus.argtypes = [P, i64, i32, P, P, P, P]
    L.vss_step_versus.restype = ctypes.c_int
    L.vss_reset_dones_replay.argtypes = [P, i64, P, P, P]
    L.vss_reset_dones_replay.restype = ctypes.c_int
    L.vss_rollout.argtypes = [P, i64, i32, P, P, P]
    L.vss_rollout.restype = ctypes.c_int
    L.vss_reset_dones.argtypes = [P, i64, P, P]
    L.vss_reset_dones.restype = ctypes.c_int
    L.vss_compute_observations.argtypes = [P, i64, P, P, i32]
    L.vss_compute_observations.restype = ctypes.c_int
    L.vss_mlp_packed_size.argtypes = [i32]
    L.vss_mlp_packed_size.restype = i64
    L.vss_mlp_pack.argtypes = [P, i32, P, P, P]
    L.vss_mlp_pack.restype = ctypes.c_int
    L.vss_policy_forward.argtypes = [P, i64, i32, P, P, P, P, ctypes.c_uint64, ctypes.c_uint64] + [P] * 6
    L.vss_policy_forward.restype = ctypes.c_int
    L.vss_value_forward_masked.argtypes = [P, i64, i32, P, P, P, P, ctypes.c_uint64, ctypes.c_uint64] + [P] * 7
    L.vss_value_forward_masked.restype = ctypes.c_int
    L.vss_actor_forward.argtypes = [P, i64, i32, P, P, P, ctypes.c_uint64, ctypes.c_uint64, P, P]
    L.vss_actor_forward.restype = ctypes.c_int
    L.vss_policy_sample.argtypes = [P, i64, i32, P, P, ctypes.c_uint64, ctypes.c_uint64, P, P, P, P]
    L.vss_policy_sample.restype = ctypes.c_int
    L.vss_actor_forward_grouped.argtypes = [P, i64, i32, P, P, ctypes.c_uint64, ctypes.c_uint64, P, P]
    L.vss_actor_forward_grouped.restype = ctypes.c_int
    L.vss_policy_sample_grouped.argtypes = [P, i64, i32, P, P, ctypes.c_uint64, ctypes.c_uint64, P]
    L.vss_policy_sample_grouped.restype = ctypes.c_int
    L.vss_match_tally.argtypes = [P, i64, i32, i64, i32, P, P, P, P]
    L.vss_match_tally.restype = ctypes.c_int
    L.vss_episode_stats.argtypes = [P, i64] + [P] * 7
    L.vss_episode_stats.restype = ctypes.c_int
    L.vss_tanh_grad_chunks.argtypes = [i64, i32]
    L.vss_tanh_grad_chunks.restype = i64
    L.vss_tanh_grad_bias.argtypes = [P, i64, i32, P, P, P, P]
    L.vss_tanh_grad_bias.restype = ctypes.c_int
    L.vss_linear_tanh.argtypes = [P, i64, i32, i32, P, P, P, P]
    L.vss_linear_tanh.restype = ctypes.c_int
    L.vss_linear_tanh_out.argtypes = [P, i64, i32, i32, P, P, P, P, i32, P, P]
    L.vss_linear_tanh_out.restype = ctypes.c_int
    L.vss_linear_tanh_backward_chunks.argtypes = [i64, i32, i32]
    L.vss_linear_tanh_backward_chunks.restype = i64
    L.vss_linear_tanh_backward.argtypes = [P, i64, i32, i32, P, P, P, P, P]
    L.vss_linear_tanh_backward.restype = ctypes.c_int
    L.vss_output_backward_chunks.argtypes = [i64, i32, i32]
    L.vss_output_backward_chunks.restype = i64
    L.vss_output_backward.argtypes = [P, i64, i32, i32, P, P, P, P, P, P]
    L.vss_output_backward.restype = ctypes.c_int
    L.vss_linear_tanh_bf16x6.argtypes = [P, i64, i32, i32, P, P, P, P, P]
    L.vss_linear_tanh_bf16x6.restype = ctypes.c_int
    L.vss_linear_tanh_out_bf16x6.argtypes = [P, i64, i32, i32, P, P, P, P, i32, P, P, P]
    L.vss_linear_tanh_out_bf16x6.restype = ctypes.c_int
    L.vss_linear_tanh_backward_chunks_bf16x6.argtypes = [i64, i32, i32]
    L.vss_linear_tanh_backward_chunks_bf16x6.restype = i64
    L.vss_linear_tanh_backward_bf16x6.argtypes = [P, i64, i32, i32, P, P, P, P, P, P]
    L.vss_linear_tanh_backward_bf16x6.restype = ctypes.c_int
    L.vss_weight_grad_chunks_bf16x6.argtypes = [i64, i32, i32]
    L.vss_weight_grad_chunks_bf16x6.restype = i64
    L.vss_weight_grad_bf16x6.argtypes = [P, i64, i32, i32, P, P, P]
    L.vss_weight_grad_bf16x6.restype = ctypes.c_int
    L.vss_first_weight_grad_chunks_bf16x6.argtypes = [i64, i32, i32]
    L.vss_first_weight_grad_chunks_bf16x6.restype = i64
    L.vss_first_weight_grad_bf16x6.argtypes = [P, i64, i32, i32, P, P, P]
    L.vss_first_weight_grad_bf16x6.restype = ctypes.c_int
    L.vss_weight_planes_bf16x6.argtypes = [P, i32, P, P, P, P, P]
    L.vss_weight_planes_bf16x6.restype = ctypes.c_int
    f32 = ctypes.c_float
    L.vss_ppo_loss_scratch_floats.argtypes = [i64, i32]
    L.vss_ppo_loss_scratch_floats.restype = i64
    L.vss_ppo_loss.argtypes = [P, i64, i64, i32] + [P] * 8 + [f32] * 5 + [i32] + [P] * 6
    L.vss_ppo_loss.restype = ctypes.c_int
    L.vss_grad_sq_partials_count.argtypes = [i64]
    L.vss_grad_sq_partials_count.restype = i64
    L.vss_grad_sq_partials.argtypes = [P, i64, P, P]
    L.vss_grad_sq_partials.restype = ctypes.c_int
    L.vss_adam_step_clipped.argtypes = [P, i64, i32, P] + [f32] * 5 + [i64] + [P] * 5
    L.vss_adam_step_clipped.restype = ctypes.c_int
    L.vss_sum_parts.argtypes = [P, i32] + [P] * 8
    L.vss_sum_parts.restype = ctypes.c_int
    L.vss_output_backward_direct_chunks.argtypes = [i64, i32, i32]
    L.vss_output_backward_direct_chunks.restype = i64
    L.vss_output_backward_direct.argtypes = [P, i64, i32, i32, P, P, P, P, P, P]
    L.vss_output_backward_direct.restype = ctypes.c_int
    L.vss_ppo_loss_direct_scratch_floats.argtypes = [i64, i32]
    L.vss_ppo_loss_direct_scratch_floats.restype = i64
    L.vss_ppo_loss_direct.argtypes = ([P, i64, i64, i32, P, i32, P, P, i32, P] + [P] * 4 + [P, i32, ctypes.c_double]
                                      + [P, P] + [f32] * 5 + [i32] + [P] * 8)
    L.vss_ppo_loss_direct.restype = ctypes.c_int
    L.vss_minibatch_gather_parts.argtypes = [i64]
    L.vss_minibatch_gather_parts.restype = i64
    L.vss_minibatch_gather.argtypes = [P, i64, i64, i64, P, i64, i64] + [P] * 13
    L.vss_minibatch_gather.restype = ctypes.c_int
    L.vss_adv_part_sum.argtypes = [P, i32, P, P]
    L.vss_adv_part_sum.restype = ctypes.c_int
    L.vss_first_layer_bf16x6.argtypes = [P, i64, i32, i32, P, P, P, P]
    L.vss_first_layer_bf16x6.restype = ctypes.c_int
    L.vss_linear_tanh_loss_blocks_bf16x6.argtypes = [i64, i32, i32]
    L.vss_linear_tanh_loss_blocks_bf16x6.restype = i64
    L.vss_linear_tanh_loss_bf16x6.argtypes = ([P, i32, i64, i64, i32, i32, P, P, i32, P, P] + [P] * 4
                                              + [i32, ctypes.c_double] + [P] * 3 + [f32] * 4 + [i32] + [P] * 5)
    L.vss_linear_tanh_loss_bf16x6.restype = ctypes.c_int
    L.vss_ppo_loss_fused_finish.argtypes = [P, i64, i32, i64, P, i64, P, P, f32, f32] + [P] * 5
    L.vss_ppo_loss_fused_finish.restype = ctypes.c_int
    L.vss_randperm_scratch_bytes.argtypes = [i64]
    L.vss_randperm_scratch_bytes.restype = i64
    L.vss_randperm.argtypes = [P, i64, P, P, P, i64]
    L.vss_randperm.restype = ctypes.c_int
    L.vss_randperm_bits.argtypes = [P, i64, ctypes.c_int32, P, P, P, i64]
    L.vss_randperm_bits.restype = ctypes.c_int
    if L.vss_abi_version() != ABI_VERSION:
        raise NativeError(f"libvss_amd ABI {L.vss_abi_version()} != expected {ABI_VERSION}")
    _lib = L
    return L


def check(rc: int, what: str) -> None:
    if rc != 0:
        msg = load().vss_error_string(rc).decode()
        raise NativeError(f"{what} failed: {msg} (code {rc})")


def ptr(t: torch.Tensor | None):
    return None if t is None else t.data_ptr()


def stream_of(device: torch.device) -> int:
    return torch.cuda.current_stream(device).cuda_stream


def require_device(device) -> torch.device:
    device = torch.device(device)
    if device.type != "cuda":
        raise NativeError(f"VSS runs on a ROCm GPU (got device {device}); there is no CPU path")
    if not torch.cuda.is_available():
        raise NativeError("VSS needs a ROCm GPU but torch.cuda.is_available() is False")
    load()
    return device
```

### rsoccer-isaac-cleanrl_amd/vss_amd/minibatch.py

```python
from __future__ import annotations

import os
import warnings

import numpy as np
import torch
import torch.distributed as dist

from . import mlp as M
from .loss import (N_ACT, adv_part_sum, minibatch_gather, minibatch_gather_parts, ppo_loss, ppo_loss_direct,
                   ppo_loss_fused_finish, randperm)
from .update import (linear_tanh_loss_x6, linear_tanh_loss_x6_ok, linear_tanh_mixed, linear_tanh_out_x6,
                     output_backward_direct, output_backward_direct_ok, sum_parts, x6_ok)

FUSED_LOSS = os.environ.get("VSS_FUSED_LOSS", "1") != "0"
RANDPERM_HIP = os.environ.get("VSS_RANDPERM", "torch") == "hip"
MLP_ROW_PAD = 256
GRAPH_CHECK_REPLAY = 12
GRAPH_CHECK_FACTOR = 4

PACKET_CAPTURE = "DEBUG_CLR_GRAPH_PACKET_CAPTURE"
_SEEN_BEFORE_INIT = {"value": None, "seen": False}


def _note_packet_capture():
    if not torch.cuda.is_initialized():
        _SEEN_BEFORE_INIT["value"] = os.environ.get(PACKET_CAPTURE)
        _SEEN_BEFORE_INIT["seen"] = True


def _startup_environment_value():
    try:
        with open("/proc/self/environ", "rb") as f:
            for item in f.read().split(b"\0"):
                if item.startswith(PACKET_CAPTURE.encode() + b"="):
                    return item.split(b"=", 1)[1].decode()
    except OSError:
        pass
    return None


def disable_graph_packet_capture() -> bool:
    if PACKET_CAPTURE not in os.environ and not torch.cuda.is_initialized():
        os.environ[PACKET_CAPTURE] = "0"
    _note_packet_capture()
    return os.environ.get(PACKET_CAPTURE) == "0"


def packet_capture_off_at_init() -> bool:
    if os.environ.get(PACKET_CAPTURE) != "0":
        return False
    if _SEEN_BEFORE_INIT["seen"]:
        return _SEEN_BEFORE_INIT["value"] == "0"
    return _startup_environment_value() == "0"


_note_packet_capture()



def autocast(args, device):
    enabled = getattr(args, "amp", "none") == "bf16" and torch.device(device).type == "cuda"
    return torch.autocast(device_type="cuda", dtype=torch.bfloat16, enabled=enabled)


def normalize_advantages(mb_adv: torch.Tensor, world: int = 1, global_stats: bool = True) -> torch.Tensor:
    if world == 1 or not global_stats:
        return (mb_adv - mb_adv.mean()) / (mb_adv.std() + 1e-8)
    a = mb_adv.double()
    s = torch.stack([a.sum(), (a * a).sum(), torch.tensor(float(a.numel()), dtype=torch.float64, device=a.device)])
    dist.all_reduce(s)
    n = s[2]
    mean = s[0] / n
    std = ((s[1] - n * mean * mean) / (n - 1)).clamp(min=0).sqrt()
    return (mb_adv - mean.float()) / (std.float() + 1e-8)


def minibatch_losses(agent, args, obs, actions, logprobs, adv, returns, values):
    if getattr(args, "amp", "none") == "none":
        mean = M.mlp_forward(agent.actor_mean, obs)
        value = M.mlp_forward(agent.critic, obs)
    else:
        with autocast(args, obs.device):
            mean, value = agent.actor_mean(obs), agent.critic(obs)
        mean, value = mean.float(), value.float()
    return ppo_loss(mean, agent.actor_logstd, value, actions, logprobs, adv, returns, values, args.clip_coef,
                    args.ent_coef, args.vf_coef, args.clip_vloss)



def direct_minibatch_ok(agent, args, flat) -> bool:
    if flat is None or M.UPDATE_GEMM != "x6" or getattr(args, "amp", "none") != "none":
        return False
    for seq, outs in ((agent.actor_mean, N_ACT), (agent.critic, (1,))):
        if not M.fused_mlp_ok(seq):
            return False
        ws, _ = M.mlp_wb(seq)
        if len(ws) < 3:
            return False
        (n, k), k_out = ws[-2].shape, ws[-1].shape[0]
        if not (x6_ok(256, k, n) and n == 256 and k_out in (1, 2, 6) and k_out in outs
                and output_backward_direct_ok(k_out, n)):
            return False
    owned = {id(p) for p in flat.params}
    return all(id(p) in owned and getattr(p, "_vss_flat_grad", False) and p.grad is not None and p.grad.is_cuda
               and p.grad.dtype == torch.float32 and p.grad.is_contiguous()
               for p in agent.parameters() if p.requires_grad)


def fused_loss_ok(agent, rows_pad: int) -> bool:
    for seq in (agent.actor_mean, agent.critic):
        ws, _ = M.mlp_wb(seq)
        (n, k), k_out = ws[-2].shape, ws[-1].shape[0]
        if not linear_tanh_loss_x6_ok(rows_pad, k, n, k_out):
            return False
    return M.mlp_wb(agent.critic)[0][-1].shape[0] == 1


def direct_minibatch(agent, args, obs, act, logp, adv, adv_part, adv_count, ret, val):
    (pfa, pba), (pfc, pbc) = M.nets_planes([M.mlp_wb(agent.actor_mean)[0], M.mlp_wb(agent.critic)[0]], obs.shape[0])
    planes = {id(agent.actor_mean): (pfa, pba), id(agent.critic): (pfc, pbc)}

    def forward(seq):
        ws, bs = M.mlp_wb(seq)
        pf, pb = planes[id(seq)]
        hs = [obs]
        for layer in range(len(ws) - 2):
            hs.append(linear_tanh_mixed(hs[-1], ws[layer], bs[layer], planes=pf.get(layer)))
        y, parts = linear_tanh_out_x6(hs[-1], ws[-2], bs[-2], ws[-1], bs[-1], planes=pf.get(len(ws) - 2), parts=True)
        hs.append(y)
        return hs, ws, bs, parts, pb, [t.grad for w, b in zip(ws, bs) for t in (w, b)]

    def backward(net, g, defer):
        hs, ws, _, _, pb, d = net
        n = len(ws)
        gz, gb, _ = output_backward_direct(g, ws[-1], hs[-1], out_db=d[2 * n - 3], out_dw=d[2 * n - 2], defer=defer)
        M.backward_layers(hs, ws, pb, gz, gb, n - 2, d, [None] * (2 * n), defer)

    def fused(seq, is_actor, defer):
        ws, bs = M.mlp_wb(seq)
        pf, pb = planes[id(seq)]
        n = len(ws)
        d = [t.grad for w, b in zip(ws, bs) for t in (w, b)]
        hs = [obs]
        for layer in range(n - 2):
            hs.append(linear_tanh_mixed(hs[-1], ws[layer], bs[layer], planes=pf.get(layer)))
        role = dict(act=act, logp=logp, adv=adv, adv_part=adv_part, adv_count=adv_count,
                    logstd=agent.actor_logstd) if is_actor else dict(ret=ret, val=val)
        gz, gb, _, st = linear_tanh_loss_x6(hs[-1], ws[-2], bs[-2], ws[-1], bs[-1], logp.shape[0], is_actor,
                                            planes=pf.get(n - 2), clip_coef=args.clip_coef, vf_coef=args.vf_coef,
                                            clip_vloss=args.clip_vloss, out_db=d[2 * n - 3], out_dw=d[2 * n - 2],
                                            defer=defer, **role)
        return (hs, ws, pb, gz, gb, n, d), st

    if FUSED_LOSS and fused_loss_ok(agent, obs.shape[0]):
        with torch.no_grad():
            defer = []
            a_net, a_st = fused(agent.actor_mean, True, defer)
            c_net, c_st = fused(agent.critic, False, defer)
            loss, stats = ppo_loss_fused_finish(a_st, c_st, logp.shape[0], agent.actor_logstd, args.ent_coef,
                                                args.vf_coef, agent.actor_logstd.grad, a_net[6][-1], c_net[6][-1])
            for hs, ws, pb, gz, gb, n, d in (a_net, c_net):
                M.backward_layers(hs, ws, pb, gz, gb, n - 2, d, [None] * (2 * n), defer)
            sum_parts(defer)
        return loss, tuple(stats[i] for i in range(6))
    with torch.no_grad():
        actor, critic = forward(agent.actor_mean), forward(agent.critic)
        (_, _, ba, pa, _, da), (_, _, bc, pc, _, dc) = actor, critic
        g_mean, g_value, loss, stats = ppo_loss_direct(
            pa, ba[-1], pc, bc[-1], agent.actor_logstd, act, logp, adv, adv_part, adv_count, ret, val, args.clip_coef,
            args.ent_coef, args.vf_coef, args.clip_vloss, agent.actor_logstd.grad, da[-1], dc[-1])
        defer = []
        backward(actor, g_mean, defer)
        backward(critic, g_value, defer)
        sum_parts(defer)
    return loss, tuple(stats[i] for i in range(6))


class DirectRows:

    def __init__(self, mb: int, rows_pad: int, obs_w: int, act_w: int, device):
        z = lambda *shape, dtype=torch.float32: torch.zeros(shape, device=device, dtype=dtype)
        self.obs, self.act = z(rows_pad, obs_w), z(rows_pad, act_w)
        self.logp, self.adv, self.ret, self.val = z(mb), z(mb), z(mb), z(mb)
        self.adv_part = z(minibatch_gather_parts(mb), 2, dtype=torch.float64)
        self.adv_glob = z(1, 2, dtype=torch.float64)

    def gather(self, inds, b_obs, b_actions, b_logprobs, b_advantages, b_returns, b_values, norm_adv: bool,
               world: int = 1, global_stats: bool = True):
        minibatch_gather(inds, b_obs, b_actions, b_logprobs, b_advantages, b_returns, b_values, self.obs, self.act,
                         self.logp, self.adv, self.ret, self.val, self.adv_part)
        mb = inds.numel()
        if not norm_adv:
            return None, 0.0
        if world > 1 and global_stats:
            adv_part_sum(self.adv_part, self.adv_glob)
            dist.all_reduce(self.adv_glob)
            return self.adv_glob, float(mb * world)
        return self.adv_part, float(mb)


def padding_rows(mb: int, device) -> int:
    return (-mb) % MLP_ROW_PAD if torch.device(device).type == "cuda" else 0


def graph_check_due(replays: int) -> bool:
    r = GRAPH_CHECK_REPLAY
    while r < replays:
        r *= GRAPH_CHECK_FACTOR
    return r == replays


class MinibatchGraph:

    def __init__(self, agent, flat, args, mb, obs_dim, act_dim, device):
        self.agent, self.flat, self.args = agent, flat, args
        z = lambda *shape: torch.zeros(shape, device=device)
        mb_pad = mb + padding_rows(mb, device)
        self.direct = direct_minibatch_ok(agent, args, flat)
        if self.direct:
            self.rows = DirectRows(mb, mb_pad, int(np.prod(obs_dim)), int(np.prod(act_dim)), device)
            self.obs, self.act, self.logp = self.rows.obs, self.rows.act, self.rows.logp
            self.adv_src = None
        else:
            self.obs, self.act = z(mb_pad, *obs_dim), z(mb_pad, *act_dim)
            self.logp, self.adv, self.ret, self.val = z(mb), z(mb), z(mb), z(mb)
        self.graph = None
        self.warm = False
        self.out = None
        self.replays = 0
        self.failed = False
        self.pool = torch.cuda.MemPool() if SHARED_POOL and torch.device(device).type == "cuda" else None
        self.stream = torch.cuda.Stream(device=device) if self.pool is not None else None

    def _body(self):
        if self.direct:
            r = self.rows
            _, st = direct_minibatch(self.agent, self.args, r.obs, r.act, r.logp, r.adv, *self.adv_src, r.ret, r.val)
            return st
        loss, st = minibatch_losses(self.agent, self.args, self.obs, self.act, self.logp, self.adv, self.ret,
                                    self.val)
        self.flat.zeroed_backward(loss)
        return tuple(t.detach() for t in st)

    def _eager(self):
        if self.pool is None:
            return self._body()
        cur = torch.cuda.current_stream()
        self.stream.wait_stream(cur)
        with torch.cuda.stream(self.stream), torch.cuda.use_mem_pool(self.pool):
            out = self._body()
        cur.wait_stream(self.stream)
        return out

    def _capture(self):
        torch.cuda.synchronize()
        if self.pool is None:
            free, _ = torch.cuda.mem_get_info()
            if free < 1.25 * (torch.cuda.memory_reserved() - torch.cuda.memory_allocated()):
                torch.cuda.empty_cache()
        g = torch.cuda.CUDAGraph()
        with torch.cuda.graph(g, pool=self.pool.id if self.pool is not None else None, stream=self.stream,
                              capture_error_mode="thread_local"):
            self.out = self._body()
        self.graph = g

    def run(self, inds, inds_pad, b_obs, b_actions, b_logprobs, mb_adv, b_returns, b_values):
        if inds.numel() != self.logp.numel() or inds_pad.numel() != self.obs.shape[0] or \
                b_obs.shape[1:] != self.obs.shape[1:] or b_actions.shape[1:] != self.act.shape[1:]:
            raise ValueError(f"MinibatchGraph: minibatch {inds.numel()} (+{inds_pad.numel() - inds.numel()} padding) "
                             f"x {tuple(b_obs.shape[1:])} does not match the captured "
                             f"{self.logp.numel()} (+{self.obs.shape[0] - self.logp.numel()}) x {tuple(self.obs.shape[1:])}")
        torch.index_select(b_obs, 0, inds_pad, out=self.obs)
        torch.index_select(b_actions, 0, inds_pad, out=self.act)
        torch.index_select(b_logprobs, 0, inds, out=self.logp)
        torch.index_select(b_returns, 0, inds, out=self.ret)
        torch.index_select(b_values, 0, inds, out=self.val)
        self.adv.copy_(mb_adv)
        return self._step()

    def run_direct(self, inds, b_obs, b_actions, b_logprobs, b_advantages, b_returns, b_values, world: int = 1):
        if inds.numel() != self.logp.numel() or b_obs[0].numel() != self.obs.shape[1] or \
                b_actions[0].numel() != self.act.shape[1]:
            raise ValueError(f"MinibatchGraph: minibatch {inds.numel()} x {tuple(b_obs.shape[1:])} does not match the "
                             f"captured {self.logp.numel()} x {self.obs.shape[1]}")
        src = self.rows.gather(inds, b_obs, b_actions, b_logprobs, b_advantages, b_returns, b_values,
                               self.args.norm_adv, world, getattr(self.args, "global_adv_norm", True))
        if self.graph is not None and (src[0] is not self.adv_src[0] or src[1] != self.adv_src[1]):
            raise ValueError("MinibatchGraph: the advantage normalisation changed after the capture")
        self.adv_src = src
        return self._step()

    def prepare(self, b_obs, b_actions, b_logprobs, b_advantages, b_returns, b_values, world: int = 1):
        if not self.direct or self.graph is not None or self.failed:
            return
        mb = self.logp.numel()
        inds = torch.arange(mb, device=self.logp.device)
        self.adv_src = self.rows.gather(inds, b_obs, b_actions, b_logprobs, b_advantages, b_returns, b_values,
                                        self.args.norm_adv, world, getattr(self.args, "global_adv_norm", True))
        self.warm = True
        self._eager()
        self._capture()
        self.flat.zero()
        torch.cuda.synchronize()

    def _step(self):
        if self.failed:
            return self._eager()
        if self.graph is None:
            if not self.warm:
                self.warm = True
                return self._eager()
            self._capture()
        self.graph.replay()
        self.replays += 1
        if graph_check_due(self.replays):
            return self._check()
        return self.out

    def _check(self):
        got = [t.clone() for t in self.out] + [self.flat.flat.clone()]
        want = list(self._eager())
        same = all(torch.equal(a, b) for a, b in zip(got, want + [self.flat.flat]))
        if same:
            return self.out
        warnings.warn(f"MinibatchGraph: replay {self.replays} differs from the eager minibatch; the update runs "
                      f"eagerly from here on ({PACKET_CAPTURE}={os.environ.get(PACKET_CAPTURE, '<unset>')})",
                      RuntimeWarning)
        self.failed, self.graph = True, None
        return tuple(want)


SHARED_POOL = os.environ.get("VSS_SHARED_POOL", "1") != "0"
_WARNED_PACKET_CAPTURE = [False]


def make_minibatch_graph(agent, flat, args, batch, obs_dim, act_dim, device):
    mb = batch // args.num_minibatches
    if not getattr(args, "update_graph", False) or torch.device(device).type != "cuda" or \
            getattr(args, "amp", "none") != "none" or batch % mb:
        return None
    if not packet_capture_off_at_init():
        if not _WARNED_PACKET_CAPTURE[0]:
            warnings.warn(f"{PACKET_CAPTURE}={os.environ.get(PACKET_CAPTURE, '<unset>')}: the runtime did not "
                          "provably start with graph packet capture off, so the update minibatches run eagerly (call "
                          "disable_graph_packet_capture() before anything initialises the GPU)", RuntimeWarning)
            _WARNED_PACKET_CAPTURE[0] = True
        return None
    return MinibatchGraph(agent, flat, args, mb, obs_dim, act_dim, device)


_SIDE_STREAMS = {}


class EpochPermutations:

    def __init__(self, batch: int, device, gen, epochs: int, ahead: bool = True):
        self.batch, self.device, self.gen, self.left = batch, torch.device(device), gen, epochs
        self.side = None
        if ahead and self.device.type == "cuda":
            key = self.device.index if self.device.index is not None else torch.cuda.current_device()
            self.side = _SIDE_STREAMS.setdefault(key, torch.cuda.Stream(device=self.device))
        self.pending = None

    def _perm(self):
        if self.device.type != "cuda" or not RANDPERM_HIP or self.batch >= 2 ** 31:
            return torch.randperm(self.batch, device=self.device, generator=self.gen)
        seed = torch.randint(-2 ** 63, 2 ** 63 - 1, (1,), device=self.device, dtype=torch.int64, generator=self.gen)
        return randperm(self.batch, seed)

    def _draw(self):
        self.left -= 1
        if self.side is None:
            return self._perm(), None
        main = torch.cuda.current_stream(self.device)
        self.side.wait_stream(main)
        with torch.cuda.stream(self.side):
            p = self._perm()
            ev = torch.cuda.Event()
            ev.record(self.side)
        return p, ev

    def next(self) -> torch.Tensor:
        p, ev = self.pending if self.pending is not None else self._draw()
        self.pending = None
        if ev is not None:
            torch.cuda.current_stream(self.device).wait_event(ev)
            p.record_stream(torch.cuda.current_stream(self.device))
        if self.side is not None and self.left > 0:
            self.pending = self._draw()
        return p


def warmup_kernels(args, train) -> float:
    import copy
    import random
    import time
    t0 = time.perf_counter()
    rng = (random.getstate(), np.random.get_state(), torch.get_rng_state(),
           torch.cuda.get_rng_state_all() if torch.cuda.is_available() else None)
    w = copy.copy(args)
    w.num_envs = 3 * 16384 if args.env_id == "dma" else 16384
    w.num_steps, w.num_updates, w.total_timesteps = 8, 1, 0
    w.log, w.evaluate, w.capture_video, w.track, w.kernel_warmup = False, False, False, False, False
    w.batch_size = int(w.num_envs * w.num_steps)
    w.minibatch_size = int(w.batch_size // w.num_minibatches)
    train(w)
    random.setstate(rng[0])
    np.random.set_state(rng[1])
    torch.set_rng_state(rng[2])
    if rng[3] is not None:
        torch.cuda.set_rng_state_all(rng[3])
        torch.cuda.synchronize()
    return time.perf_counter() - t0


__all__ = ["FUSED_LOSS", "RANDPERM_HIP", "MLP_ROW_PAD", "GRAPH_CHECK_REPLAY", "GRAPH_CHECK_FACTOR", "PACKET_CAPTURE",
           "disable_graph_packet_capture", "packet_capture_off_at_init", "autocast", "normalize_advantages",
           "minibatch_losses", "direct_minibatch_ok", "fused_loss_ok", "direct_minibatch", "DirectRows",
           "padding_rows", "graph_check_due", "MinibatchGraph", "make_minibatch_graph", "EpochPermutations",
           "warmup_kernels"]
```

### rsoccer-isaac-cleanrl_amd/vss_amd/update.py

```python
from __future__ import annotations

import ctypes

import torch

from . import _native as N

_COLS = (64, 128, 256, 512, 1024)


def tanh_grad_bias(gy: torch.Tensor, y: torch.Tensor):
    if gy.shape != y.shape or gy.dim() != 2:
        raise ValueError(f"gy {tuple(gy.shape)} and y {tuple(y.shape)} must be the same (rows, cols)")
    if gy.device.type != "cuda":
        gz = gy * (1.0 - y * y)
        return gz, gz.sum(0)
    rows, cols = y.shape
    if cols not in _COLS or gy.dtype != torch.float32 or y.dtype != torch.float32:
        raise ValueError(f"vss_tanh_grad_bias: fp32 with cols in {_COLS}, got {gy.dtype}/{y.dtype} x {cols}")
    lib = N.load()
    if rows == 0:
        return torch.empty_like(y), torch.zeros(cols, device=y.device, dtype=torch.float32)
    gy = gy.contiguous()
    y = y.contiguous()
    gz = torch.empty_like(y)
    partial = torch.empty((lib.vss_tanh_grad_chunks(rows, cols), cols), device=y.device, dtype=torch.float32)
    N.check(lib.vss_tanh_grad_bias(N.stream_of(y.device), rows, cols, gy.data_ptr(), y.data_ptr(), gz.data_ptr(),
                                   partial.data_ptr()), "vss_tanh_grad_bias")
    return gz, partial.sum(0)


def gemm_shape_ok(k: int, n: int) -> bool:
    return k >= 4 and k % 4 == 0 and n >= 128 and n % 128 == 0


def _fp32_2d(name, *ts):
    for t in ts:
        if t.dtype != torch.float32:
            raise ValueError(f"{name}: fp32 tensors only, got {t.dtype}")


def _out(out, shape, like):
    if out is None:
        return torch.empty(shape, device=like.device, dtype=torch.float32)
    if tuple(out.shape) != tuple(shape) or out.dtype != torch.float32 or not out.is_contiguous():
        raise ValueError(f"out must be a contiguous fp32 {tuple(shape)} tensor, got {out.dtype} {tuple(out.shape)}")
    return out


SUM_PARTS_MAX = 512


def _reduce_parts(parts: torch.Tensor, out: torch.Tensor | None, defer: list | None) -> torch.Tensor:
    if defer is not None and parts.is_cuda and parts.shape[0] <= SUM_PARTS_MAX:
        if out is None:
            out = torch.empty(parts.shape[1:], device=parts.device, dtype=torch.float32)
        defer.append((parts, out))
        return out
    return torch.sum(parts, 0, out=out)


def sum_parts(jobs) -> None:
    jobs = sorted(jobs, key=lambda j: -j[0].shape[0])
    for q0 in range(0, len(jobs), 32):
        chunk = jobs[q0:q0 + 32]
        cols = {k: [] for k in ("src", "dst", "parts", "pstride", "rows", "cols", "sld", "dld")}
        for parts, out in chunk:
            try:
                p3 = parts.view(parts.shape[0], -1, parts.shape[-1]) if parts.dim() >= 2 else None
                o2 = out.view(1, -1) if out.dim() == 1 else out
            except RuntimeError as e:
                raise ValueError(f"sum_parts: parts {tuple(parts.shape)} / out {tuple(out.shape)} are not "
                                 f"viewable in the launch's shape ({e})") from None
            if p3 is None or parts.dtype != torch.float32 or out.dtype != torch.float32 or o2.dim() != 2 \
                    or tuple(p3.shape[1:]) != tuple(o2.shape) or p3.stride(2) != 1 or o2.stride(1) != 1 \
                    or not parts.is_cuda or out.device != parts.device:
                raise ValueError(f"sum_parts: parts {tuple(parts.shape)} / out {tuple(out.shape)}")
            cols["src"].append(p3.data_ptr())
            cols["dst"].append(o2.data_ptr())
            cols["parts"].append(p3.shape[0])
            cols["pstride"].append(p3.stride(0))
            cols["rows"].append(o2.shape[0])
            cols["cols"].append(o2.shape[1])
            cols["sld"].append(p3.stride(1) if o2.shape[0] > 1 else o2.shape[1])
            cols["dld"].append(o2.stride(0) if o2.shape[0] > 1 else o2.shape[1])
        c = len(chunk)
        Pa, I64 = ctypes.c_void_p * c, ctypes.c_int64 * c
        N.check(N.load().vss_sum_parts(N.stream_of(chunk[0][0].device), c, Pa(*cols["src"]), Pa(*cols["dst"]),
                                       I64(*cols["parts"]), I64(*cols["pstride"]), I64(*cols["rows"]),
                                       I64(*cols["cols"]), I64(*cols["sld"]), I64(*cols["dld"])), "vss_sum_parts")


def linear_tanh(x: torch.Tensor, w: torch.Tensor, b: torch.Tensor, out: torch.Tensor | None = None) -> torch.Tensor:
    if x.dim() != 2 or w.dim() != 2 or x.shape[1] != w.shape[1] or b.shape != (w.shape[0],):
        raise ValueError(f"linear_tanh: x {tuple(x.shape)}, w {tuple(w.shape)}, b {tuple(b.shape)}")
    if x.device.type != "cuda":
        return torch.addmm(b, x, w.t()).tanh_()
    rows, k = x.shape
    n = w.shape[0]
    _fp32_2d("vss_linear_tanh", x, w, b)
    if not gemm_shape_ok(k, n):
        raise ValueError(f"vss_linear_tanh: k % 4 == 0 and n % 128 == 0 required, got k={k}, n={n}")
    lib = N.load()
    y = _out(out, (rows, n), x)
    if rows == 0:
        return y
    x, w, b = x.contiguous(), w.contiguous(), b.contiguous()
    N.check(lib.vss_linear_tanh(N.stream_of(x.device), rows, k, n, x.data_ptr(), w.data_ptr(), b.data_ptr(),
                                y.data_ptr()), "vss_linear_tanh")
    return y


def linear_tanh_out_ok(rows: int, k: int, n: int, k_out: int) -> bool:
    return n == 256 and rows > 0 and rows % 256 == 0 and k % 64 == 0 and k_out in (1, 2, 6)


def linear_tanh_out(x: torch.Tensor, w: torch.Tensor, b: torch.Tensor, w_out: torch.Tensor, b_out: torch.Tensor):
    rows, k = x.shape
    n, k_out = w.shape[0], w_out.shape[0]
    if x.device.type != "cuda":
        y = torch.addmm(b, x, w.t()).tanh_()
        return y, torch.addmm(b_out, y, w_out.t())
    if w.shape != (n, k) or b.shape != (n,) or w_out.shape != (k_out, n) or b_out.shape != (k_out,) \
            or not linear_tanh_out_ok(rows, k, n, k_out):
        raise ValueError(f"linear_tanh_out: x {tuple(x.shape)}, w {tuple(w.shape)}, w_out {tuple(w_out.shape)}")
    _fp32_2d("vss_linear_tanh_out", x, w, b, w_out, b_out)
    x, w, b, w_out = x.contiguous(), w.contiguous(), b.contiguous(), w_out.contiguous()
    y = torch.empty((rows, n), device=x.device, dtype=torch.float32)
    part = torch.empty((n // 64, rows, k_out), device=x.device, dtype=torch.float32)
    N.check(N.load().vss_linear_tanh_out(N.stream_of(x.device), rows, k, n, x.data_ptr(), w.data_ptr(), b.data_ptr(),
                                         y.data_ptr(), k_out, w_out.data_ptr(), part.data_ptr()), "vss_linear_tanh_out")
    return y, part.sum(0).add_(b_out)


def linear_tanh_backward(gz_next: torch.Tensor, w_next: torch.Tensor, y: torch.Tensor, out: torch.Tensor | None = None):
    if gz_next.dim() != 2 or w_next.dim() != 2 or y.dim() != 2 or gz_next.shape[0] != y.shape[0] \
            or w_next.shape != (gz_next.shape[1], y.shape[1]):
        raise ValueError(f"linear_tanh_backward: gz_next {tuple(gz_next.shape)}, w_next {tuple(w_next.shape)}, "
                         f"y {tuple(y.shape)}")
    if gz_next.device.type != "cuda":
        gz = gz_next.mm(w_next) * (1.0 - y * y)
        return gz, gz.sum(0)
    rows, k_next = gz_next.shape
    n = y.shape[1]
    _fp32_2d("vss_linear_tanh_backward", gz_next, w_next, y)
    if not gemm_shape_ok(k_next, n):
        raise ValueError(f"vss_linear_tanh_backward: k_next % 4 == 0 and n % 128 == 0 required, got {k_next}, {n}")
    lib = N.load()
    gz = _out(out, (rows, n), y)
    if rows == 0:
        return gz, torch.zeros(n, device=y.device, dtype=torch.float32)
    gz_next, y = gz_next.contiguous(), y.contiguous()
    w_t = w_next.t().contiguous()
    partial = torch.empty((lib.vss_linear_tanh_backward_chunks(rows, k_next, n), n), device=y.device,
                          dtype=torch.float32)
    N.check(lib.vss_linear_tanh_backward(N.stream_of(y.device), rows, k_next, n, gz_next.data_ptr(), w_t.data_ptr(),
                                         y.data_ptr(), gz.data_ptr(), partial.data_ptr()),
            "vss_linear_tanh_backward")
    return gz, partial.sum(0)


def output_backward_ok(k_out: int, n: int) -> bool:
    return 1 <= k_out <= 8 and n >= 128 and n % 128 == 0 and 1024 % n == 0


def output_backward(g_out: torch.Tensor, w_out: torch.Tensor, y: torch.Tensor, out_db: torch.Tensor | None = None,
                    out_dw: torch.Tensor | None = None, defer: list | None = None):
    if g_out.dim() != 2 or w_out.dim() != 2 or y.dim() != 2 or g_out.shape[0] != y.shape[0] \
            or w_out.shape != (g_out.shape[1], y.shape[1]):
        raise ValueError(f"output_backward: g_out {tuple(g_out.shape)}, w_out {tuple(w_out.shape)}, y {tuple(y.shape)}")
    if g_out.device.type != "cuda":
        gz = g_out.mm(w_out) * (1.0 - y * y)
        return gz, gz.sum(0), g_out.t().mm(y)
    rows, k_out = g_out.shape
    n = y.shape[1]
    _fp32_2d("vss_output_backward", g_out, w_out, y)
    if not output_backward_ok(k_out, n):
        raise ValueError(f"vss_output_backward: k_out <= 8 and n in (128, 256, 512, 1024) required, got {k_out}, {n}")
    lib = N.load()
    k_pad = 4 if k_out <= 4 else 8
    gz = torch.empty((rows, n), device=y.device, dtype=torch.float32)
    if rows == 0:
        z = torch.zeros(n, device=y.device, dtype=torch.float32)
        return gz, z, torch.zeros((k_out, n), device=y.device, dtype=torch.float32)
    g_pad = torch.nn.functional.pad(g_out, (0, k_pad - k_out)).contiguous()
    w_t = torch.nn.functional.pad(w_out, (0, 0, 0, k_pad - k_out)).t().contiguous()
    y = y.contiguous()
    chunks = lib.vss_output_backward_chunks(rows, k_pad, n)
    bpart = torch.empty((chunks, n), device=y.device, dtype=torch.float32)
    wpart = torch.empty((chunks, k_pad, n), device=y.device, dtype=torch.float32)
    N.check(lib.vss_output_backward(N.stream_of(y.device), rows, k_pad, n, g_pad.data_ptr(), w_t.data_ptr(),
                                    y.data_ptr(), gz.data_ptr(), bpart.data_ptr(), wpart.data_ptr()),
            "vss_output_backward")
    return gz, _reduce_parts(bpart, out_db, defer), _reduce_parts(wpart[:, :k_out], out_dw, defer)


def output_backward_direct_ok(k_out: int, n: int) -> bool:
    return k_out in (1, 2, 3, 4, 6, 8) and n >= 128 and n % 128 == 0 and 1024 % n == 0


def output_backward_direct(g_out: torch.Tensor, w_out: torch.Tensor, y: torch.Tensor, out_db: torch.Tensor | None = None,
                           out_dw: torch.Tensor | None = None, defer: list | None = None):
    rows, k_out = g_out.shape
    n = y.shape[1]
    if w_out.shape != (k_out, n) or y.shape[0] != rows or not output_backward_direct_ok(k_out, n):
        raise ValueError(f"output_backward_direct: g_out {tuple(g_out.shape)}, w_out {tuple(w_out.shape)}, y {tuple(y.shape)}")
    _x6_check("vss_output_backward_direct", True, g_out, w_out, y)
    lib = N.load()
    g_out, w_out, y = g_out.contiguous(), w_out.contiguous(), y.contiguous()
    gz = torch.empty((rows, n), device=y.device, dtype=torch.float32)
    chunks = lib.vss_output_backward_direct_chunks(rows, k_out, n)
    bpart = torch.empty((max(chunks, 1), n), device=y.device, dtype=torch.float32)
    wpart = torch.empty((max(chunks, 1), k_out, n), device=y.device, dtype=torch.float32)
    if rows == 0:
        bpart.zero_()
        wpart.zero_()
    N.check(lib.vss_output_backward_direct(N.stream_of(y.device), rows, k_out, n, g_out.data_ptr(), w_out.data_ptr(),
                                           y.data_ptr(), gz.data_ptr(), bpart.data_ptr(), wpart.data_ptr()),
            "vss_output_backward_direct")
    return gz, _reduce_parts(bpart, out_db, defer), _reduce_parts(wpart, out_dw, defer)


def linear_tanh_loss_x6_ok(rows_pad: int, k: int, n: int, k_out: int) -> bool:
    return n == 256 and k_out in (1, 2) and x6_ok(rows_pad, k, n)


def linear_tanh_loss_x6(x: torch.Tensor, w: torch.Tensor, b: torch.Tensor, w_out: torch.Tensor, b_out: torch.Tensor,
                        rows: int, actor: bool, *, planes: torch.Tensor | None = None, act=None, logp=None, adv=None,
                        adv_part=None, adv_count: float = 0.0, logstd=None, ret=None, val=None, clip_coef: float = 0.2,
                        vf_coef: float = 0.5, clip_vloss: bool = False, out_db=None, out_dw=None, defer=None):
    rows_pad, k = x.shape
    n, k_out = w.shape[0], w_out.shape[0]
    _x6_check("vss_linear_tanh_loss_bf16x6", w.shape == (n, k) and b.shape == (n,) and w_out.shape == (k_out, n)
              and b_out.shape == (k_out,) and 0 < rows <= rows_pad and linear_tanh_loss_x6_ok(rows_pad, k, n, k_out)
              and (actor or k_out == 1), x, w, b, w_out)
    rows_t = (act, logp, adv, logstd) if actor else (ret,) + ((val,) if clip_vloss else ())
    for t in rows_t:
        if t is None or t.dtype != torch.float32 or t.device != x.device or not t.is_contiguous():
            raise ValueError("linear_tanh_loss_x6: the role's loss inputs as contiguous fp32 tensors on the device")
    if actor and (act.shape[0] < rows_pad or act.shape[1] != k_out or logp.shape[0] < rows or adv.shape[0] < rows
                  or logstd.numel() != k_out):
        raise ValueError(f"linear_tanh_loss_x6: actor inputs for {rows} rows and {k_out} actions")
    if not actor and (ret.shape[0] < rows or (clip_vloss and val.shape[0] < rows)):
        raise ValueError(f"linear_tanh_loss_x6: critic inputs for {rows} rows")
    if adv_part is not None and (adv_part.dtype != torch.float64 or adv_part.device != x.device
                                 or adv_part.dim() != 2 or adv_part.shape[1] != 2 or not adv_part.is_contiguous()):
        raise ValueError("linear_tanh_loss_x6: adv_part must be a contiguous (parts, 2) fp64 tensor on the device")
    lib = N.load()
    x, b, w_out, b_out = x.contiguous(), b.contiguous(), w_out.contiguous(), b_out.contiguous()
    if planes is None:
        planes = weight_planes([(w.contiguous(), False)])[0]
    _, pp, keep = _w_and_planes(w, planes)
    blocks = lib.vss_linear_tanh_loss_blocks_bf16x6(rows_pad, k, n)
    f32 = dict(device=x.device, dtype=torch.float32)
    gz = torch.empty((rows_pad, n), **f32)
    part_cs = torch.empty((blocks, n), **f32)
    part_dw = torch.empty((blocks, k_out, n), **f32)
    stats = torch.empty((blocks, 32), **f32)
    ptr = lambda t: t.data_ptr() if t is not None else None
    c = float(clip_coef)
    N.check(lib.vss_linear_tanh_loss_bf16x6(
        N.stream_of(x.device), 0 if actor else 1, rows_pad, rows, k, n, x.data_ptr(), b.data_ptr(), k_out,
        w_out.data_ptr(), b_out.data_ptr(), ptr(act), ptr(logp), ptr(adv), ptr(adv_part),
        adv_part.shape[0] if adv_part is not None else 0, float(adv_count), ptr(logstd), ptr(ret),
        ptr(val) if clip_vloss else None, c, 1 - c, 1 + c, float(vf_coef), int(bool(clip_vloss)), gz.data_ptr(),
        part_cs.data_ptr(), part_dw.data_ptr(), stats.data_ptr(), pp), "vss_linear_tanh_loss_bf16x6")
    del keep
    return gz, _reduce_parts(part_cs, out_db, defer), _reduce_parts(part_dw, out_dw, defer), stats



def x6_ok(rows: int, k: int, n: int) -> bool:
    return rows > 0 and rows % 256 == 0 and n > 0 and n % 128 == 0 and n <= 4096 and k > 0 and k % 64 == 0


def x6_wgrad_ok(rows: int, n_out: int, k_in: int) -> bool:
    return rows > 0 and rows % 64 == 0 and n_out % 256 == 0 and 0 < n_out <= 4096 and k_in % 128 == 0 \
        and 0 < k_in <= 4096


def _planes(w: torch.Tensor) -> torch.Tensor:
    return torch.empty((3, w.numel()), device=w.device, dtype=torch.int16)


def weight_planes(jobs) -> list:
    if not 1 <= len(jobs) <= 16:
        raise ValueError(f"weight_planes: 1..16 weights per launch, got {len(jobs)}")
    ws, ns, ks, ts, outs = [], [], [], [], []
    for w, tr in jobs:
        if w.dim() != 2 or w.dtype != torch.float32 or not w.is_cuda or not w.is_contiguous():
            raise ValueError(f"weight_planes: contiguous fp32 ROCm (rows, cols) weights, got {w.dtype} {tuple(w.shape)}")
        n, k = (w.shape[1], w.shape[0]) if tr else (w.shape[0], w.shape[1])
        ws.append(w.data_ptr())
        ns.append(n)
        ks.append(k)
        ts.append(int(bool(tr)))
        outs.append(_planes(w))
    c = len(jobs)
    P, I = ctypes.c_void_p * c, ctypes.c_int32 * c
    N.check(N.load().vss_weight_planes_bf16x6(N.stream_of(jobs[0][0].device), c, P(*ws), I(*ns), I(*ks), I(*ts),
                                              P(*[o.data_ptr() for o in outs])), "vss_weight_planes_bf16x6")
    return outs


def _x6_check(name, cond, *ts):
    if not cond:
        raise ValueError(f"{name}: shape outside the bf16x6 kernels' exact shapes: {[tuple(t.shape) for t in ts]}")
    _fp32_2d(name, *ts)
    for t in ts:
        if t.device.type != "cuda":
            raise ValueError(f"{name}: ROCm tensors only (no CPU path)")


def _w_and_planes(w: torch.Tensor, planes: torch.Tensor | None):
    if planes is None:
        scratch = _planes(w)
        return w.data_ptr(), scratch.data_ptr(), (w, scratch)
    if planes.dtype != torch.int16 or planes.numel() != 3 * w.numel():
        raise ValueError(f"planes: weight_planes() output of this weight, got {planes.dtype} {tuple(planes.shape)}")
    return None, planes.data_ptr(), (planes,)


def linear_tanh_x6(x: torch.Tensor, w: torch.Tensor, b: torch.Tensor, out: torch.Tensor | None = None,
                   planes: torch.Tensor | None = None) -> torch.Tensor:
    rows, k = x.shape
    n = w.shape[0]
    _x6_check("vss_linear_tanh_bf16x6", w.shape == (n, k) and b.shape == (n,) and x6_ok(rows, k, n), x, w, b)
    x, w, b = x.contiguous(), w.contiguous(), b.contiguous()
    y = _out(out, (rows, n), x)
    wp, pp, keep = _w_and_planes(w, planes)
    N.check(N.load().vss_linear_tanh_bf16x6(N.stream_of(x.device), rows, k, n, x.data_ptr(), wp,
                                            b.data_ptr(), y.data_ptr(), pp), "vss_linear_tanh_bf16x6")
    del keep
    return y


def linear_tanh_out_x6(x: torch.Tensor, w: torch.Tensor, b: torch.Tensor, w_out: torch.Tensor, b_out: torch.Tensor,
                       out: torch.Tensor | None = None, planes: torch.Tensor | None = None, parts: bool = False):
    rows, k = x.shape
    n, k_out = w.shape[0], w_out.shape[0]
    _x6_check("vss_linear_tanh_out_bf16x6", w.shape == (n, k) and b.shape == (n,) and w_out.shape == (k_out, n)
              and b_out.shape == (k_out,) and n == 256 and k_out in (1, 2, 6) and x6_ok(rows, k, n), x, w, b, w_out)
    x, w, b, w_out = x.contiguous(), w.contiguous(), b.contiguous(), w_out.contiguous()
    y = _out(out, (rows, n), x)
    part = torch.empty((n // 64, rows, k_out), device=x.device, dtype=torch.float32)
    wp, pp, keep = _w_and_planes(w, planes)
    N.check(N.load().vss_linear_tanh_out_bf16x6(N.stream_of(x.device), rows, k, n, x.data_ptr(), wp,
                                                b.data_ptr(), y.data_ptr(), k_out, w_out.data_ptr(), part.data_ptr(),
                                                pp), "vss_linear_tanh_out_bf16x6")
    del keep
    if parts:
        return y, part
    return y, part.sum(0).add_(b_out)


def linear_tanh_backward_x6(gz_next: torch.Tensor, w_next: torch.Tensor, y: torch.Tensor,
                            out: torch.Tensor | None = None, out_db: torch.Tensor | None = None,
                            planes: torch.Tensor | None = None, defer: list | None = None):
    rows, k_next = gz_next.shape
    n = y.shape[1]
    _x6_check("vss_linear_tanh_backward_bf16x6", w_next.shape == (k_next, n) and y.shape[0] == rows
              and x6_ok(rows, k_next, n), gz_next, w_next, y)
    lib = N.load()
    gz_next, y = gz_next.contiguous(), y.contiguous()
    if planes is None:
        wp, pp, keep = _w_and_planes(w_next.t().contiguous(), None)
    else:
        wp, pp, keep = _w_and_planes(w_next, planes)
    gz = _out(out, (rows, n), y)
    partial = torch.empty((lib.vss_linear_tanh_backward_chunks_bf16x6(rows, k_next, n), n), device=y.device,
                          dtype=torch.float32)
    N.check(lib.vss_linear_tanh_backward_bf16x6(N.stream_of(y.device), rows, k_next, n, gz_next.data_ptr(),
                                                wp, y.data_ptr(), gz.data_ptr(), partial.data_ptr(), pp),
            "vss_linear_tanh_backward_bf16x6")
    del keep
    return gz, _reduce_parts(partial, out_db, defer)


def weight_grad_x6(grad: torch.Tensor, x: torch.Tensor, out: torch.Tensor | None = None,
                   defer: list | None = None) -> torch.Tensor:
    rows, n_out = grad.shape
    k_in = x.shape[1]
    _x6_check("vss_weight_grad_bf16x6", x.shape[0] == rows and x6_wgrad_ok(rows, n_out, k_in), grad, x)
    lib = N.load()
    grad, x = grad.contiguous(), x.contiguous()
    parts = torch.empty((lib.vss_weight_grad_chunks_bf16x6(rows, n_out, k_in), n_out, k_in), device=x.device,
                        dtype=torch.float32)
    N.check(lib.vss_weight_grad_bf16x6(N.stream_of(x.device), rows, n_out, k_in, grad.data_ptr(), x.data_ptr(),
                                       parts.data_ptr()), "vss_weight_grad_bf16x6")
    return _reduce_parts(parts, out, defer)


def first_layer_x6_ok(k: int, n: int) -> bool:
    return n == 256 and 0 < k <= 64 and k % 4 == 0


def first_layer_x6(x: torch.Tensor, w: torch.Tensor, b: torch.Tensor, out: torch.Tensor | None = None) -> torch.Tensor:
    rows, k = x.shape
    n = w.shape[0]
    _x6_check("vss_first_layer_bf16x6", w.shape == (n, k) and b.shape == (n,) and first_layer_x6_ok(k, n), x, w, b)
    x, w, b = x.contiguous(), w.contiguous(), b.contiguous()
    y = _out(out, (rows, n), x)
    N.check(N.load().vss_first_layer_bf16x6(N.stream_of(x.device), rows, k, n, x.data_ptr(), w.data_ptr(), b.data_ptr(),
                                            y.data_ptr()), "vss_first_layer_bf16x6")
    return y


def first_wgrad_ok(rows: int, n_out: int, k_in: int) -> bool:
    return rows > 0 and rows % 64 == 0 and n_out == 256 and 0 < k_in <= 64 and k_in % 4 == 0


def first_weight_grad_x6(grad: torch.Tensor, x: torch.Tensor, out: torch.Tensor | None = None,
                         defer: list | None = None) -> torch.Tensor:
    rows, n_out = grad.shape
    k_in = x.shape[1]
    _x6_check("vss_first_weight_grad_bf16x6", x.shape[0] == rows and first_wgrad_ok(rows, n_out, k_in), grad, x)
    lib = N.load()
    grad, x = grad.contiguous(), x.contiguous()
    parts = torch.empty((lib.vss_first_weight_grad_chunks_bf16x6(rows, n_out, k_in), n_out, k_in), device=x.device,
                        dtype=torch.float32)
    N.check(lib.vss_first_weight_grad_bf16x6(N.stream_of(x.device), rows, n_out, k_in, grad.data_ptr(), x.data_ptr(),
                                             parts.data_ptr()), "vss_first_weight_grad_bf16x6")
    return _reduce_parts(parts, out, defer)



def linear_tanh_mixed(x: torch.Tensor, w: torch.Tensor, b: torch.Tensor, planes: torch.Tensor | None = None) -> torch.Tensor:
    rows, k = x.shape
    n = w.shape[0]
    if x.is_cuda and rows > 0 and first_layer_x6_ok(k, n):
        return first_layer_x6(x, w, b)
    main = rows // 256 * 256
    if main == 0 or not x6_ok(main, k, n):
        return linear_tanh(x, w, b)
    y = torch.empty((rows, n), device=x.device, dtype=torch.float32)
    linear_tanh_x6(x[:main], w, b, out=y[:main], planes=planes)
    if main < rows:
        torch.addmm(b, x[main:], w.t(), out=y[main:]).tanh_()
    return y


def linear_tanh_out_mixed(x: torch.Tensor, w: torch.Tensor, b: torch.Tensor, w_out: torch.Tensor, b_out: torch.Tensor,
                          planes: torch.Tensor | None = None):
    rows, k = x.shape
    n, k_out = w.shape[0], w_out.shape[0]
    main = rows // 256 * 256
    if main == 0 or not x6_ok(main, k, n) or n != 256 or k_out not in (1, 2, 6):
        y = linear_tanh(x, w, b)
        return y, torch.addmm(b_out, y, w_out.t())
    y = torch.empty((rows, n), device=x.device, dtype=torch.float32)
    _, o_main = linear_tanh_out_x6(x[:main], w, b, w_out, b_out, out=y[:main], planes=planes)
    if main == rows:
        return y, o_main
    y_t = torch.addmm(b, x[main:], w.t(), out=y[main:]).tanh_()
    return y, torch.cat([o_main, torch.addmm(b_out, y_t, w_out.t())])


def linear_tanh_backward_mixed(gz_next: torch.Tensor, w_next: torch.Tensor, y: torch.Tensor,
                               out_db: torch.Tensor | None = None, planes: torch.Tensor | None = None,
                               defer: list | None = None):
    rows, k_next = gz_next.shape
    n = y.shape[1]
    main = rows // 256 * 256
    if main == 0 or not x6_ok(main, k_next, n):
        gz, db = linear_tanh_backward(gz_next, w_next, y)
        return gz, (db if out_db is None else out_db.copy_(db))
    gz = torch.empty((rows, n), device=y.device, dtype=torch.float32)
    _, db = linear_tanh_backward_x6(gz_next[:main], w_next, y[:main], out=gz[:main], out_db=out_db, planes=planes,
                                    defer=defer if main == rows else None)
    if main < rows:
        y_t = y[main:]
        gz_t = torch.mm(gz_next[main:], w_next, out=gz[main:]).mul_(1.0 - y_t * y_t)
        db = db.add_(gz_t.sum(0)) if out_db is not None else db + gz_t.sum(0)
    return gz, db


def weight_grad_mixed(grad: torch.Tensor, x: torch.Tensor, out: torch.Tensor | None = None,
                      defer: list | None = None) -> torch.Tensor:
    rows, n_out = grad.shape
    k_in = x.shape[1]
    main = rows // 64 * 64
    if main > 0 and first_wgrad_ok(main, n_out, k_in):
        fn = first_weight_grad_x6
    elif main > 0 and x6_wgrad_ok(main, n_out, k_in):
        fn = weight_grad_x6
    else:
        return torch.mm(grad.t(), x, out=out)
    dw = fn(grad[:main], x[:main], out=out, defer=defer if main == rows else None)
    if main < rows:
        dw = dw.addmm_(grad[main:].t(), x[main:])
    return dw
```

Measured before the change: 1.696 billion env-steps/s.

## Run MLP PPO update in row bands with accumulating GEMM epilogues

Adds a banded training path that runs the whole forward, loss and backward for each MLP in row bands. Activations and gradients stay in band-sized scratch buffers, and weight, bias and loss partials are accumulated in place through new ACC template variants of the GEMM kernels. The aim is to keep per-band intermediates cache-resident and cut full-minibatch activation memory traffic. The cost is more kernel launches per band, plus read-modify-write traffic on the partial buffers.

```diff
diff --git a/include/vss.h b/include/vss.h
--- a/include/vss.h
+++ b/include/vss.h
@@ -7,7 +7,7 @@
 extern "C" {
 #endif
 
-#define VSS_ABI_VERSION 2
+#define VSS_ABI_VERSION 3
 
 #define VSS_NUM_TEAMS 2
 #define VSS_NUM_ROBOTS 3
@@ -208,6 +208,53 @@
 int vss_first_weight_grad_bf16x6(void* stream, int64_t rows, int32_t n_out, int32_t k_in, const float* grad,
                                  const float* x, float* partial);
 
+int vss_weight_grad_acc_bf16x6(void* stream, int64_t rows, int32_t n_out, int32_t k_in, const float* grad,
+                               const float* x, float* partial, int32_t accumulate);
+int vss_first_weight_grad_acc_bf16x6(void* stream, int64_t rows, int32_t n_out, int32_t k_in, const float* grad,
+                                     const float* x, float* partial, int32_t accumulate);
+int vss_linear_tanh_backward_acc_bf16x6(void* stream, int64_t rows, int32_t k_next, int32_t n_out,
+                                        const float* grad_next, const float* w_next_t, const float* y, float* grad_in,
+                                        float* bias_partial, uint16_t* w_split, int32_t accumulate);
+int vss_linear_tanh_loss_acc_bf16x6(void* stream, int32_t role, int64_t rows_pad, int64_t rows, int64_t loss_rows,
+                                    int32_t k_in, int32_t n_out, const float* x, const float* bias, int32_t k_out,
+                                    const float* w_out, const float* b_out, const float* action, const float* logprob_old,
+                                    const float* adv, const double* adv_part, int32_t adv_nparts, double adv_count,
+                                    const float* logstd, const float* returns, const float* values_old, float clip_coef,
+                                    float clip_lo, float clip_hi, float vf_coef, int32_t clip_vloss, float* grad_in,
+                                    float* part_cs, float* part_dwo, float* part_stats, const uint16_t* w_split,
+                                    int32_t accumulate);
+
+#define VSS_MLP_MAX_LAYERS 8
+typedef struct vss_mlp_net {
+  int32_t layers, role;
+  int32_t width[VSS_MLP_MAX_LAYERS + 1];
+  const float* w[VSS_MLP_MAX_LAYERS];
+  const float* bias[VSS_MLP_MAX_LAYERS];
+  const uint16_t* planes_f[VSS_MLP_MAX_LAYERS];
+  const uint16_t* planes_b[VSS_MLP_MAX_LAYERS];
+} vss_mlp_net;
+typedef struct vss_mlp_rows {
+  const float *obs, *action, *logprob_old, *adv;
+  const double* adv_part;
+  int32_t adv_nparts;
+  double adv_count;
+  const float *logstd, *returns, *values_old;
+  float clip_coef, clip_lo, clip_hi, vf_coef;
+  int32_t clip_vloss;
+} vss_mlp_rows;
+typedef struct vss_mlp_scratch {
+  float* h[VSS_MLP_MAX_LAYERS];
+  float* gz[VSS_MLP_MAX_LAYERS];
+} vss_mlp_scratch;
+typedef struct vss_mlp_parts {
+  float* wgrad[VSS_MLP_MAX_LAYERS];
+  float* bias[VSS_MLP_MAX_LAYERS];
+  float *dwo, *stats;
+} vss_mlp_parts;
+int vss_mlp_train_banded_bf16x6(void* stream, const vss_mlp_net* net, const vss_mlp_rows* rows_in, int64_t rows,
+                                int64_t rows_pad, int64_t band_rows, const vss_mlp_scratch* scratch,
+                                const vss_mlp_parts* parts);
+
 int64_t vss_ppo_loss_scratch_floats(int64_t rows_pad, int32_t n_act);
 int vss_ppo_loss(void* stream, int64_t rows, int64_t rows_pad, int32_t n_act, const float* mean, const float* logstd,
                  const float* value, const float* action, const float* logprob_old, const float* adv,
diff --git a/rsoccer-isaac-cleanrl_amd/csrc/vss_gemm_x6.hip b/rsoccer-isaac-cleanrl_amd/csrc/vss_gemm_x6.hip
--- a/rsoccer-isaac-cleanrl_amd/csrc/vss_gemm_x6.hip
+++ b/rsoccer-isaac-cleanrl_amd/csrc/vss_gemm_x6.hip
@@ -314,7 +314,7 @@
   return lane_sel(m3, c[0], c[1]);
 }
 
-template <int EPI, int SP, int SQ, class C, int KO = 0>
+template <int EPI, int SP, int SQ, class C, int KO = 0, bool ACC = false>
 __global__ __launch_bounds__(C::THREADS, C::BPC) void gemm_x6_kernel(Args a) {
   constexpr int BI = C::BI, BJ = C::BJ, TI = C::TI, TJ = C::TJ, PJ = C::PJ;
   constexpr bool PDMA = SP == ST_DMA;
@@ -715,6 +715,11 @@
           }
           acc[i][j] = v;
         } else {
+          if constexpr (ACC) {
+            const f32x4 old = *reinterpret_cast<const f32x4*>(a.out + ((int64_t)sp * a.nj * BJ + jg) * a.ldo + ig);
+#pragma unroll
+            for (int r = 0; r < 4; ++r) v[r] += old[r];
+          }
           *reinterpret_cast<f32x4*>(a.out + ((int64_t)sp * a.nj * BJ + jg) * a.ldo + ig) = v;
         }
       }
@@ -768,6 +773,7 @@
       float t = epi_lds[E_CS + f];
 #pragma unroll
       for (int m = 1; m < C::WJ; ++m) t += epi_lds[E_CS + m * BI + f];
+      if constexpr (ACC) t += a.part_cs[(int64_t)slot * BI + f];
       a.part_cs[(int64_t)slot * BI + f] = t;
     }
     for (int x = tid; x < KO * BI; x += C::THREADS) {
@@ -775,9 +781,15 @@
       float t = epi_lds[E_DW + o * BI + f];
 #pragma unroll
       for (int m = 1; m < C::WJ; ++m) t += epi_lds[E_DW + (m * KO + o) * BI + f];
+      if constexpr (ACC) t += a.part_dwo[((int64_t)slot * KO + o) * BI + f];
       a.part_dwo[((int64_t)slot * KO + o) * BI + f] = t;
     }
-    if (tid < kLossStats) a.part_stats[(int64_t)slot * kLossStats + tid] = epi_lds[E_ST + tid] + epi_lds[E_ST + kLossStats + tid];
+    if constexpr (ACC) {
+      if (tid < kLossStats)
+        a.part_stats[(int64_t)slot * kLossStats + tid] += epi_lds[E_ST + tid] + epi_lds[E_ST + kLossStats + tid];
+    } else {
+      if (tid < kLossStats) a.part_stats[(int64_t)slot * kLossStats + tid] = epi_lds[E_ST + tid] + epi_lds[E_ST + kLossStats + tid];
+    }
   }
   if constexpr (EPI == EPI_DTANH) {
     __syncthreads();
@@ -785,6 +797,7 @@
       float t = epi_lds[f];
 #pragma unroll
       for (int m = 1; m < C::WJ; ++m) t += epi_lds[m * BI + f];
+      if constexpr (ACC) t += a.partial[(int64_t)(slot / a.ni) * (a.ni * BI) + it0 * BI + f];
       a.partial[(int64_t)(slot / a.ni) * (a.ni * BI) + it0 * BI + f] = t;
     }
   }
@@ -802,6 +815,7 @@
   return rho * 256 + 16 * ((phi >> 3) ^ kswz(rho)) + 8 * ((phi >> 2) & 1);
 }
 
+template <bool ACC>
 __global__ __launch_bounds__(FW_THREADS, 1) void first_wgrad_kernel(int64_t kpairs, int32_t k_in, const float* __restrict__ grad,
                                                                       const float* __restrict__ x, float* __restrict__ partial) {
   __shared__ __attribute__((aligned(16))) char lds[2 * FW_BUF];
@@ -931,7 +945,10 @@
 #pragma unroll
       for (int i = 0; i < 4; ++i)
 #pragma unroll
-        for (int r = 0; r < 4; ++r) partial[((int64_t)b * FW_N + 64 * fs + 16 * i + 4 * fg + r) * k_in + c] = acc[i][j][r];
+        for (int r = 0; r < 4; ++r) {
+          if constexpr (ACC) partial[((int64_t)b * FW_N + 64 * fs + 16 * i + 4 * fg + r) * k_in + c] += acc[i][j][r];
+          else partial[((int64_t)b * FW_N + 64 * fs + 16 * i + 4 * fg + r) * k_in + c] = acc[i][j][r];
+        }
     }
   }
 }
@@ -998,14 +1015,14 @@
   return p;
 }
 
-template <int EPI, int SP, int SQ, class C, int KO = 0>
+template <int EPI, int SP, int SQ, class C, int KO = 0, bool ACC = false>
 static int launch(void* stream, Args a, const Plan& pl) {
   a.ni = pl.ni;
   a.nj = pl.nj;
   a.kpairs = pl.kpairs;
   a.items = pl.items;
   a.splits = pl.splits;
-  hipLaunchKernelGGL((gemm_x6_kernel<EPI, SP, SQ, C, KO>), dim3((unsigned)pl.grid), dim3(C::THREADS), 0,
+  hipLaunchKernelGGL((gemm_x6_kernel<EPI, SP, SQ, C, KO, ACC>), dim3((unsigned)pl.grid), dim3(C::THREADS), 0,
                      (hipStream_t)stream, a);
   return hipGetLastError() == hipSuccess ? VSS_OK : VSS_E_LAUNCH;
 }
@@ -1163,17 +1180,19 @@
   return fb_plan<CfgB>(rows, k_in, n_out).grid;
 }
 
-int vss_linear_tanh_loss_bf16x6(void* stream, int32_t role, int64_t rows_pad, int64_t rows, int32_t k_in, int32_t n_out,
-                                const float* x, const float* bias, int32_t k_out, const float* w_out, const float* b_out,
-                                const float* action, const float* logprob_old, const float* adv, const double* adv_part,
-                                int32_t adv_nparts, double adv_count, const float* logstd, const float* returns,
-                                const float* values_old, float clip_coef, float clip_lo, float clip_hi, float vf_coef,
-                                int32_t clip_vloss, float* grad_in, float* part_cs, float* part_dwo, float* part_stats,
-                                const uint16_t* w_split) {
+int vss_linear_tanh_loss_acc_bf16x6(void* stream, int32_t role, int64_t rows_pad, int64_t rows, int64_t loss_rows,
+                                    int32_t k_in, int32_t n_out, const float* x, const float* bias, int32_t k_out,
+                                    const float* w_out, const float* b_out, const float* action, const float* logprob_old,
+                                    const float* adv, const double* adv_part, int32_t adv_nparts, double adv_count,
+                                    const float* logstd, const float* returns, const float* values_old, float clip_coef,
+                                    float clip_lo, float clip_hi, float vf_coef, int32_t clip_vloss, float* grad_in,
+                                    float* part_cs, float* part_dwo, float* part_stats, const uint16_t* w_split,
+                                    int32_t accumulate) {
   using namespace vx6;
   using C = CfgB;
   const bool actor = role == 0;
   if ((role != 0 && role != 1) || n_out != 256 || !fb_shape_ok<C>(rows_pad, k_in, n_out) || rows <= 0 || rows > rows_pad ||
+      loss_rows < rows || (accumulate != 0 && accumulate != 1) ||
       misaligned(x) || misaligned(grad_in) || misaligned(w_split) || !bias || !w_out || !b_out || !part_cs || !part_dwo ||
       !part_stats || (actor && (k_out < 1 || k_out > 2 || !action || !logprob_old || !adv || !logstd ||
                                 (adv_part && (adv_nparts < 1 || !(adv_count > 1.0))))) ||
@@ -1196,16 +1215,34 @@
   a.clip_lo = clip_lo;
   a.clip_hi = clip_hi;
   a.vf_coef = vf_coef;
-  a.inv_n = 1.0f / (float)rows;
+  a.inv_n = 1.0f / (float)loss_rows;
   a.clip_vloss = clip_vloss;
   a.rows_real = rows;
   a.part_cs = part_cs;
   a.part_dwo = part_dwo;
   a.part_stats = part_stats;
   const Plan pl = fb_plan<C>(rows_pad, k_in, n_out);
+  if (accumulate) {
+    if (!actor) return launch<EPI_LOSS_C, ST_DMA, ST_ROW, C, 1, true>(stream, a, pl);
+    if (k_out == 1) return launch<EPI_LOSS_A, ST_DMA, ST_ROW, C, 1, true>(stream, a, pl);
+    return launch<EPI_LOSS_A, ST_DMA, ST_ROW, C, 2, true>(stream, a, pl);
+  }
   if (!actor) return launch<EPI_LOSS_C, ST_DMA, ST_ROW, C, 1>(stream, a, pl);
   if (k_out == 1) return launch<EPI_LOSS_A, ST_DMA, ST_ROW, C, 1>(stream, a, pl);
   return launch<EPI_LOSS_A, ST_DMA, ST_ROW, C, 2>(stream, a, pl);
+}
+
+int vss_linear_tanh_loss_bf16x6(void* stream, int32_t role, int64_t rows_pad, int64_t rows, int32_t k_in, int32_t n_out,
+                                const float* x, const float* bias, int32_t k_out, const float* w_out, const float* b_out,
+                                const float* action, const float* logprob_old, const float* adv, const double* adv_part,
+                                int32_t adv_nparts, double adv_count, const float* logstd, const float* returns,
+                                const float* values_old, float clip_coef, float clip_lo, float clip_hi, float vf_coef,
+                                int32_t clip_vloss, float* grad_in, float* part_cs, float* part_dwo, float* part_stats,
+                                const uint16_t* w_split) {
+  return vss_linear_tanh_loss_acc_bf16x6(stream, role, rows_pad, rows, rows, k_in, n_out, x, bias, k_out, w_out, b_out,
+                                         action, logprob_old, adv, adv_part, adv_nparts, adv_count, logstd, returns,
+                                         values_old, clip_coef, clip_lo, clip_hi, vf_coef, clip_vloss, grad_in, part_cs,
+                                         part_dwo, part_stats, w_split, 0);
 }
 
 int64_t vss_linear_tanh_backward_chunks_bf16x6(int64_t rows, int32_t k_next, int32_t n_out) {
@@ -1218,13 +1255,14 @@
   });
 }
 
-int vss_linear_tanh_backward_bf16x6(void* stream, int64_t rows, int32_t k_next, int32_t n_out, const float* grad_next,
-                                    const float* w_next_t, const float* y, float* grad_in, float* bias_partial,
-                                    uint16_t* w_split) {
+int vss_linear_tanh_backward_acc_bf16x6(void* stream, int64_t rows, int32_t k_next, int32_t n_out,
+                                        const float* grad_next, const float* w_next_t, const float* y, float* grad_in,
+                                        float* bias_partial, uint16_t* w_split, int32_t accumulate) {
   using namespace vx6;
   return with_fb_cfg(n_out, [&](auto cfg) {
     using C = decltype(cfg);
-    if (!fb_shape_ok<C>(rows, k_next, n_out) || misaligned(grad_next) || (w_next_t && misaligned(w_next_t)) ||
+    if (!fb_shape_ok<C>(rows, k_next, n_out) || (accumulate != 0 && accumulate != 1) || misaligned(grad_next) ||
+        (w_next_t && misaligned(w_next_t)) ||
         misaligned(y) || misaligned(grad_in) || misaligned(bias_partial) || misaligned(w_split))
       return (int)VSS_E_ARG;
     int rc = w_next_t ? split_weight<C>(stream, w_next_t, n_out, k_next, w_split) : VSS_OK;
@@ -1232,8 +1270,16 @@
     Args a = fb_args(k_next, n_out, w_split, grad_next, grad_in);
     a.y = y;
     a.partial = bias_partial;
+    if (accumulate) return launch<EPI_DTANH, ST_DMA, ST_ROW, C, 0, true>(stream, a, fb_plan<C>(rows, k_next, n_out));
     return launch<EPI_DTANH, ST_DMA, ST_ROW, C>(stream, a, fb_plan<C>(rows, k_next, n_out));
   });
+}
+
+int vss_linear_tanh_backward_bf16x6(void* stream, int64_t rows, int32_t k_next, int32_t n_out, const float* grad_next,
+                                    const float* w_next_t, const float* y, float* grad_in, float* bias_partial,
+                                    uint16_t* w_split) {
+  return vss_linear_tanh_backward_acc_bf16x6(stream, rows, k_next, n_out, grad_next, w_next_t, y, grad_in, bias_partial,
+                                             w_split, 0);
 }
 
 int vss_weight_planes_bf16x6(void* stream, int32_t count, const float* const* w, const int32_t* n, const int32_t* k,
@@ -1263,10 +1309,12 @@
   return wg_plan(rows, n_out, k_in).splits;
 }
 
-int vss_weight_grad_bf16x6(void* stream, int64_t rows, int32_t n_out, int32_t k_in, const float* grad, const float* x,
-                           float* partial) {
+int vss_weight_grad_acc_bf16x6(void* stream, int64_t rows, int32_t n_out, int32_t k_in, const float* grad, const float* x,
+                               float* partial, int32_t accumulate) {
   using namespace vx6;
-  if (!wg_shape_ok(rows, n_out, k_in) || misaligned(grad) || misaligned(x) || misaligned(partial)) return VSS_E_ARG;
+  if (!wg_shape_ok(rows, n_out, k_in) || misaligned(grad) || misaligned(x) || misaligned(partial) ||
+      (accumulate != 0 && accumulate != 1))
+    return VSS_E_ARG;
   Args a{};
   a.ldp = k_in;
   a.ldq = n_out;
@@ -1274,7 +1322,13 @@
   a.q = grad;
   a.ldo = k_in;
   a.out = partial;
+  if (accumulate) return launch<EPI_WGRAD, ST_KROW, ST_KROW, CfgA, 0, true>(stream, a, wg_plan(rows, n_out, k_in));
   return launch<EPI_WGRAD, ST_KROW, ST_KROW, CfgA>(stream, a, wg_plan(rows, n_out, k_in));
+}
+
+int vss_weight_grad_bf16x6(void* stream, int64_t rows, int32_t n_out, int32_t k_in, const float* grad, const float* x,
+                           float* partial) {
+  return vss_weight_grad_acc_bf16x6(stream, rows, n_out, k_in, grad, x, partial, 0);
 }
 
 int64_t vss_first_weight_grad_chunks_bf16x6(int64_t rows, int32_t n_out, int32_t k_in) {
@@ -1285,15 +1339,25 @@
   return fw_parts(rows);
 }
 
+int vss_first_weight_grad_acc_bf16x6(void* stream, int64_t rows, int32_t n_out, int32_t k_in, const float* grad,
+                                     const float* x, float* partial, int32_t accumulate) {
+  using namespace vx6;
+  if (vss_first_weight_grad_chunks_bf16x6(rows, n_out, k_in) < 0 || misaligned(grad) || misaligned(x) || !partial ||
+      (accumulate != 0 && accumulate != 1))
+    return VSS_E_ARG;
+  const int g = fw_parts(rows);
+  if (accumulate)
+    hipLaunchKernelGGL(first_wgrad_kernel<true>, dim3((unsigned)g), dim3(FW_THREADS), 0, (hipStream_t)stream,
+                       (int64_t)(rows / (2 * KT)), k_in, grad, x, partial);
+  else
+    hipLaunchKernelGGL(first_wgrad_kernel<false>, dim3((unsigned)g), dim3(FW_THREADS), 0, (hipStream_t)stream,
+                       (int64_t)(rows / (2 * KT)), k_in, grad, x, partial);
+  return hipGetLastError() == hipSuccess ? VSS_OK : VSS_E_LAUNCH;
+}
+
 int vss_first_weight_grad_bf16x6(void* stream, int64_t rows, int32_t n_out, int32_t k_in, const float* grad,
                                  const float* x, float* partial) {
-  using namespace vx6;
-  if (vss_first_weight_grad_chunks_bf16x6(rows, n_out, k_in) < 0 || misaligned(grad) || misaligned(x) || !partial)
-    return VSS_E_ARG;
-  const int g = fw_parts(rows);
-  hipLaunchKernelGGL(first_wgrad_kernel, dim3((unsigned)g), dim3(FW_THREADS), 0, (hipStream_t)stream,
-                     (int64_t)(rows / (2 * KT)), k_in, grad, x, partial);
-  return hipGetLastError() == hipSuccess ? VSS_OK : VSS_E_LAUNCH;
+  return vss_first_weight_grad_acc_bf16x6(stream, rows, n_out, k_in, grad, x, partial, 0);
 }
 
 int vss_first_layer_bf16x6(void* stream, int64_t rows, int32_t k_in, int32_t n_out, const float* x, const float* w,
@@ -1310,4 +1374,54 @@
   return hipGetLastError() == hipSuccess ? VSS_OK : VSS_E_LAUNCH;
 }
 
-}
+int vss_mlp_train_banded_bf16x6(void* stream, const vss_mlp_net* net, const vss_mlp_rows* in, int64_t rows,
+                                int64_t rows_pad, int64_t band_rows, const vss_mlp_scratch* sc,
+                                const vss_mlp_parts* pt) {
+  if (!net || !in || !sc || !pt) return VSS_E_ARG;
+  const int L = net->layers;
+  if (L < 3 || L > VSS_MLP_MAX_LAYERS || rows <= 0 || rows > rows_pad || rows_pad % 256 || rows_pad - rows >= 256 ||
+      band_rows < 256 || band_rows % 256 || !in->obs || !pt->dwo || !pt->stats || !net->w[0] || !net->w[L - 1])
+    return VSS_E_ARG;
+  const int32_t* wd = net->width;
+  for (int l = 0; l <= L - 2; ++l) {
+    if (!net->bias[l] || !sc->gz[l] || !pt->wgrad[l] || !pt->bias[l]) return VSS_E_ARG;
+    if (l >= 1 && (!net->planes_f[l] || !net->planes_b[l] || !sc->h[l])) return VSS_E_ARG;
+  }
+  if (!net->bias[L - 1]) return VSS_E_ARG;
+  const int k_out = wd[L];
+  const bool actor = net->role == 0;
+  for (int64_t off = 0; off < rows_pad; off += band_rows) {
+    const int64_t br = rows_pad - off < band_rows ? rows_pad - off : band_rows;
+    const int64_t real = rows - off < br ? rows - off : br;
+    const int acc = off > 0;
+    int rc;
+    const float* x0 = in->obs + off * wd[0];
+    rc = vss_first_layer_bf16x6(stream, br, wd[0], wd[1], x0, net->w[0], net->bias[0], sc->h[1]);
+    if (rc != VSS_OK) return rc;
+    for (int l = 1; l <= L - 3; ++l) {
+      rc = vss_linear_tanh_bf16x6(stream, br, wd[l], wd[l + 1], sc->h[l], nullptr, net->bias[l], sc->h[l + 1],
+                                  const_cast<uint16_t*>(net->planes_f[l]));
+      if (rc != VSS_OK) return rc;
+    }
+    rc = vss_linear_tanh_loss_acc_bf16x6(
+        stream, net->role, br, real, rows, wd[L - 2], wd[L - 1], sc->h[L - 2], net->bias[L - 2], k_out, net->w[L - 1],
+        net->bias[L - 1], actor ? in->action + off * k_out : nullptr, actor ? in->logprob_old + off : nullptr,
+        actor ? in->adv + off : nullptr, in->adv_part, in->adv_nparts, in->adv_count, in->logstd,
+        !actor && in->returns ? in->returns + off : nullptr, !actor && in->values_old ? in->values_old + off : nullptr,
+        in->clip_coef, in->clip_lo, in->clip_hi, in->vf_coef, in->clip_vloss, sc->gz[L - 2], pt->bias[L - 2], pt->dwo,
+        pt->stats, net->planes_f[L - 2], acc);
+    if (rc != VSS_OK) return rc;
+    for (int l = L - 2; l >= 1; --l) {
+      rc = vss_weight_grad_acc_bf16x6(stream, br, wd[l + 1], wd[l], sc->gz[l], sc->h[l], pt->wgrad[l], acc);
+      if (rc != VSS_OK) return rc;
+      rc = vss_linear_tanh_backward_acc_bf16x6(stream, br, wd[l + 1], wd[l], sc->gz[l], nullptr, sc->h[l], sc->gz[l - 1],
+                                               pt->bias[l - 1], const_cast<uint16_t*>(net->planes_b[l]), acc);
+      if (rc != VSS_OK) return rc;
+    }
+    rc = vss_first_weight_grad_acc_bf16x6(stream, br, wd[1], wd[0], sc->gz[0], x0, pt->wgrad[0], acc);
+    if (rc != VSS_OK) return rc;
+  }
+  return VSS_OK;
+}
+
+}
diff --git a/rsoccer-isaac-cleanrl_amd/vss_amd/_native.py b/rsoccer-isaac-cleanrl_amd/vss_amd/_native.py
--- a/rsoccer-isaac-cleanrl_amd/vss_amd/_native.py
+++ b/rsoccer-isaac-cleanrl_amd/vss_amd/_native.py
@@ -32,7 +32,7 @@
            os.path.join(CSRC, "vss_loss_row.h"), HEADER,
            os.path.join(CSRC, "Makefile"))
 
-ABI_VERSION = 2
+ABI_VERSION = 3
 MODE_FULL, MODE_SA, MODE_CMA, MODE_DMA = 0, 1, 2, 3
 STATE_CHANNELS = 58
 CH_BALL_X, CH_BALL_Y, CH_BALL_VX, CH_BALL_VY = 0, 1, 2, 3
@@ -52,7 +52,9 @@
             "vss_output_backward_direct_chunks", "vss_output_backward_direct", "vss_ppo_loss_direct_scratch_floats",
             "vss_ppo_loss_direct", "vss_minibatch_gather_parts", "vss_minibatch_gather", "vss_adv_part_sum",
             "vss_first_layer_bf16x6", "vss_linear_tanh_loss_blocks_bf16x6", "vss_linear_tanh_loss_bf16x6",
-            "vss_ppo_loss_fused_finish", "vss_randperm_scratch_bytes", "vss_randperm", "vss_randperm_bits")
+            "vss_ppo_loss_fused_finish", "vss_randperm_scratch_bytes", "vss_randperm", "vss_randperm_bits",
+            "vss_weight_grad_acc_bf16x6", "vss_first_weight_grad_acc_bf16x6", "vss_linear_tanh_backward_acc_bf16x6",
+            "vss_linear_tanh_loss_acc_bf16x6", "vss_mlp_train_banded_bf16x6")
 
 
 class VssParams(ctypes.Structure):
@@ -88,6 +90,32 @@
 class VssActorGroups(ctypes.Structure):
     _fields_ = [("count", ctypes.c_int32), ("group_rows", ctypes.c_int64),
                 ("actor_packed", ctypes.c_void_p * MAX_ACTOR_GROUPS), ("logstd", ctypes.c_void_p * MAX_ACTOR_GROUPS)]
+
+
+MLP_MAX_LAYERS = 8
+
+
+class VssMlpNet(ctypes.Structure):
+    _fields_ = [("layers", ctypes.c_int32), ("role", ctypes.c_int32), ("width", ctypes.c_int32 * (MLP_MAX_LAYERS + 1)),
+                ("w", ctypes.c_void_p * MLP_MAX_LAYERS), ("bias", ctypes.c_void_p * MLP_MAX_LAYERS),
+                ("planes_f", ctypes.c_void_p * MLP_MAX_LAYERS), ("planes_b", ctypes.c_void_p * MLP_MAX_LAYERS)]
+
+
+class VssMlpRows(ctypes.Structure):
+    _fields_ = [("obs", ctypes.c_void_p), ("action", ctypes.c_void_p), ("logprob_old", ctypes.c_void_p),
+                ("adv", ctypes.c_void_p), ("adv_part", ctypes.c_void_p), ("adv_nparts", ctypes.c_int32),
+                ("adv_count", ctypes.c_double), ("logstd", ctypes.c_void_p), ("returns", ctypes.c_void_p),
+                ("values_old", ctypes.c_void_p), ("clip_coef", ctypes.c_float), ("clip_lo", ctypes.c_float),
+                ("clip_hi", ctypes.c_float), ("vf_coef", ctypes.c_float), ("clip_vloss", ctypes.c_int32)]
+
+
+class VssMlpScratch(ctypes.Structure):
+    _fields_ = [("h", ctypes.c_void_p * MLP_MAX_LAYERS), ("gz", ctypes.c_void_p * MLP_MAX_LAYERS)]
+
+
+class VssMlpParts(ctypes.Structure):
+    _fields_ = [("wgrad", ctypes.c_void_p * MLP_MAX_LAYERS), ("bias", ctypes.c_void_p * MLP_MAX_LAYERS),
+                ("dwo", ctypes.c_void_p), ("stats", ctypes.c_void_p)]
 
 
 class VssRolloutIO(ctypes.Structure):
@@ -246,6 +274,18 @@
     L.vss_linear_tanh_loss_bf16x6.argtypes = ([P, i32, i64, i64, i32, i32, P, P, i32, P, P] + [P] * 4
                                               + [i32, ctypes.c_double] + [P] * 3 + [f32] * 4 + [i32] + [P] * 5)
     L.vss_linear_tanh_loss_bf16x6.restype = ctypes.c_int
+    L.vss_weight_grad_acc_bf16x6.argtypes = [P, i64, i32, i32, P, P, P, i32]
+    L.vss_weight_grad_acc_bf16x6.restype = ctypes.c_int
+    L.vss_first_weight_grad_acc_bf16x6.argtypes = [P, i64, i32, i32, P, P, P, i32]
+    L.vss_first_weight_grad_acc_bf16x6.restype = ctypes.c_int
+    L.vss_linear_tanh_backward_acc_bf16x6.argtypes = [P, i64, i32, i32, P, P, P, P, P, P, i32]
+    L.vss_linear_tanh_backward_acc_bf16x6.restype = ctypes.c_int
+    L.vss_linear_tanh_loss_acc_bf16x6.argtypes = ([P, i32, i64, i64, i64, i32, i32, P, P, i32, P, P] + [P] * 4
+                                                  + [i32, ctypes.c_double] + [P] * 3 + [f32] * 4 + [i32] + [P] * 5
+                                                  + [i32])
+    L.vss_linear_tanh_loss_acc_bf16x6.restype = ctypes.c_int
+    L.vss_mlp_train_banded_bf16x6.argtypes = [P, P, P, i64, i64, i64, P, P]
+    L.vss_mlp_train_banded_bf16x6.restype = ctypes.c_int
     L.vss_ppo_loss_fused_finish.argtypes = [P, i64, i32, i64, P, i64, P, P, f32, f32] + [P] * 5
     L.vss_ppo_loss_fused_finish.restype = ctypes.c_int
     L.vss_randperm_scratch_bytes.argtypes = [i64]
diff --git a/rsoccer-isaac-cleanrl_amd/vss_amd/minibatch.py b/rsoccer-isaac-cleanrl_amd/vss_amd/minibatch.py
--- a/rsoccer-isaac-cleanrl_amd/vss_amd/minibatch.py
+++ b/rsoccer-isaac-cleanrl_amd/vss_amd/minibatch.py
@@ -10,12 +10,14 @@
 from . import mlp as M
 from .loss import (N_ACT, adv_part_sum, minibatch_gather, minibatch_gather_parts, ppo_loss, ppo_loss_direct,
                    ppo_loss_fused_finish, randperm)
-from .update import (linear_tanh_loss_x6, linear_tanh_loss_x6_ok, linear_tanh_mixed, linear_tanh_out_x6,
-                     output_backward_direct, output_backward_direct_ok, sum_parts, x6_ok)
+from .update import (linear_tanh_loss_x6, linear_tanh_loss_x6_ok, linear_tanh_mixed, linear_tanh_out_x6, mlp_banded_ok,
+                     mlp_train_banded, output_backward_direct, output_backward_direct_ok, sum_parts, x6_ok)
 
 FUSED_LOSS = os.environ.get("VSS_FUSED_LOSS", "1") != "0"
 RANDPERM_HIP = os.environ.get("VSS_RANDPERM", "torch") == "hip"
 MLP_ROW_PAD = 256
+DEFAULT_BAND_ROWS = 0
+UPDATE_BAND_ROWS = int(os.environ.get("VSS_UPDATE_BAND_ROWS", str(DEFAULT_BAND_ROWS)))
 GRAPH_CHECK_REPLAY = 12
 GRAPH_CHECK_FACTOR = 4
 
@@ -117,6 +119,11 @@
     return M.mlp_wb(agent.critic)[0][-1].shape[0] == 1
 
 
+def update_band_rows(rows_pad: int) -> int:
+    band = -(-UPDATE_BAND_ROWS // MLP_ROW_PAD) * MLP_ROW_PAD
+    return band if 0 < band and 2 * band <= rows_pad else rows_pad
+
+
 def direct_minibatch(agent, args, obs, act, logp, adv, adv_part, adv_count, ret, val):
     (pfa, pba), (pfc, pbc) = M.nets_planes([M.mlp_wb(agent.actor_mean)[0], M.mlp_wb(agent.critic)[0]], obs.shape[0])
     planes = {id(agent.actor_mean): (pfa, pba), id(agent.critic): (pfc, pbc)}
@@ -153,6 +160,26 @@
                                             defer=defer, **role)
         return (hs, ws, pb, gz, gb, n, d), st
 
+    def banded(seq, is_actor, defer):
+        ws, bs = M.mlp_wb(seq)
+        pf, pb = planes[id(seq)]
+        role = dict(act=act, logp=logp, adv=adv, adv_part=adv_part, adv_count=adv_count,
+                    logstd=agent.actor_logstd) if is_actor else dict(ret=ret, val=val)
+        return mlp_train_banded(ws, bs, pf, pb, obs, logp.shape[0], update_band_rows(obs.shape[0]), is_actor,
+                                clip_coef=args.clip_coef, vf_coef=args.vf_coef, clip_vloss=args.clip_vloss, defer=defer,
+                                **role)
+
+    if FUSED_LOSS and fused_loss_ok(agent, obs.shape[0]) and \
+            all(mlp_banded_ok(M.mlp_wb(seq)[0], *planes[id(seq)]) for seq in (agent.actor_mean, agent.critic)):
+        with torch.no_grad():
+            defer = []
+            a_st = banded(agent.actor_mean, True, defer)
+            c_st = banded(agent.critic, False, defer)
+            loss, stats = ppo_loss_fused_finish(a_st, c_st, logp.shape[0], agent.actor_logstd, args.ent_coef,
+                                                args.vf_coef, agent.actor_logstd.grad, M.mlp_wb(agent.actor_mean)[1][-1].grad,
+                                                M.mlp_wb(agent.critic)[1][-1].grad)
+            sum_parts(defer)
+        return loss, tuple(stats[i] for i in range(6))
     if FUSED_LOSS and fused_loss_ok(agent, obs.shape[0]):
         with torch.no_grad():
             defer = []
@@ -417,6 +444,7 @@
 
 __all__ = ["FUSED_LOSS", "RANDPERM_HIP", "MLP_ROW_PAD", "GRAPH_CHECK_REPLAY", "GRAPH_CHECK_FACTOR", "PACKET_CAPTURE",
            "disable_graph_packet_capture", "packet_capture_off_at_init", "autocast", "normalize_advantages",
-           "minibatch_losses", "direct_minibatch_ok", "fused_loss_ok", "direct_minibatch", "DirectRows",
+           "minibatch_losses", "direct_minibatch_ok", "fused_loss_ok", "DEFAULT_BAND_ROWS", "UPDATE_BAND_ROWS",
+           "update_band_rows", "direct_minibatch", "DirectRows",
            "padding_rows", "graph_check_due", "MinibatchGraph", "make_minibatch_graph", "EpochPermutations",
            "warmup_kernels"]
diff --git a/rsoccer-isaac-cleanrl_amd/vss_amd/update.py b/rsoccer-isaac-cleanrl_amd/vss_amd/update.py
--- a/rsoccer-isaac-cleanrl_amd/vss_amd/update.py
+++ b/rsoccer-isaac-cleanrl_amd/vss_amd/update.py
@@ -425,6 +425,95 @@
 
 
 
+def mlp_banded_ok(ws, planes_f: dict, planes_b: dict) -> bool:
+    n = len(ws)
+    wd = [ws[0].shape[1]] + [w.shape[0] for w in ws]
+    if not 3 <= n <= N.MLP_MAX_LAYERS or not first_layer_x6_ok(wd[0], wd[1]) or not first_wgrad_ok(256, wd[1], wd[0]) \
+            or not linear_tanh_loss_x6_ok(256, wd[n - 2], wd[n - 1], wd[n]):
+        return False
+    for layer in range(1, n - 1):
+        if not (x6_ok(256, wd[layer], wd[layer + 1]) and x6_ok(256, wd[layer + 1], wd[layer])
+                and x6_wgrad_ok(256, wd[layer + 1], wd[layer]) and planes_f.get(layer) is not None
+                and planes_b.get(layer) is not None):
+            return False
+    return True
+
+
+def mlp_train_banded(ws, bs, planes_f: dict, planes_b: dict, obs: torch.Tensor, rows: int, band_rows: int, actor: bool,
+                     *, act=None, logp=None, adv=None, adv_part=None, adv_count: float = 0.0, logstd=None, ret=None,
+                     val=None, clip_coef: float = 0.2, vf_coef: float = 0.5, clip_vloss: bool = False, defer: list,
+                     scratch: dict | None = None, alias_gz: bool = True):
+    n = len(ws)
+    rows_pad = obs.shape[0]
+    wd = [ws[0].shape[1]] + [w.shape[0] for w in ws]
+    band = min(int(band_rows), rows_pad)
+    rows_t = (act, logp, adv, logstd) if actor else (ret,) + ((val,) if clip_vloss else ())
+    if any(t is None or t.dtype != torch.float32 or t.device != obs.device or not t.is_contiguous() for t in rows_t) \
+            or obs.dtype != torch.float32 or not obs.is_cuda or not obs.is_contiguous() or obs.shape[1] != wd[0] \
+            or band < 256 or band % 256 or rows_pad % 256 or not 0 < rows <= rows_pad or rows_pad - rows >= 256 \
+            or not mlp_banded_ok(ws, planes_f, planes_b) \
+            or (actor and (act.shape[0] < rows_pad or act.shape[1] != wd[n] or logp.shape[0] < rows or adv.shape[0] < rows
+                           or logstd.numel() != wd[n])) \
+            or (not actor and (wd[n] != 1 or ret.shape[0] < rows or (clip_vloss and val.shape[0] < rows))) \
+            or (adv_part is not None and (adv_part.dtype != torch.float64 or adv_part.device != obs.device
+                                          or adv_part.dim() != 2 or adv_part.shape[1] != 2
+                                          or not adv_part.is_contiguous())):
+        raise ValueError(f"mlp_train_banded: widths {wd}, obs {tuple(obs.shape)}, {rows} rows, bands of {band_rows}")
+    lib = N.load()
+    f32 = dict(device=obs.device, dtype=torch.float32)
+    net = N.VssMlpNet(layers=n, role=0 if actor else 1)
+    sc, pt = N.VssMlpScratch(), N.VssMlpParts()
+    for i, v in enumerate(wd):
+        net.width[i] = v
+    ws_c, bs_c = [w.contiguous() for w in ws], [b.contiguous() for b in bs]
+    net.w[0], net.w[n - 1] = ws_c[0].data_ptr(), ws_c[n - 1].data_ptr()
+    for layer in range(n):
+        net.bias[layer] = bs_c[layer].data_ptr()
+    if alias_gz:
+        two = [torch.empty((band, max(wd[layer + 1] for layer in range(par, n - 1, 2))), **f32) for par in (0, 1)]
+        gz = [two[layer % 2] for layer in range(n - 1)]
+    else:
+        gz = [torch.empty((band, wd[layer + 1]), **f32) for layer in range(n - 1)]
+    hs = {}
+    for layer in range(1, n - 1):
+        if planes_f[layer].dtype != torch.int16 or planes_f[layer].numel() != 3 * ws[layer].numel() \
+                or planes_b[layer].dtype != torch.int16 or planes_b[layer].numel() != 3 * ws[layer].numel():
+            raise ValueError("mlp_train_banded: planes_f / planes_b must be weight_planes() of the layers' weights")
+        net.planes_f[layer], net.planes_b[layer] = planes_f[layer].data_ptr(), planes_b[layer].data_ptr()
+        hs[layer] = torch.empty((band, wd[layer]), **f32)
+        sc.h[layer] = hs[layer].data_ptr()
+    blocks = lib.vss_linear_tanh_loss_blocks_bf16x6(band, wd[n - 2], wd[n - 1])
+    stats = torch.empty((blocks, 32), **f32)
+    dwo = torch.empty((blocks, wd[n], wd[n - 1]), **f32)
+    pt.dwo, pt.stats = dwo.data_ptr(), stats.data_ptr()
+    defer.append((dwo, ws[n - 1].grad))
+    for layer in range(n - 1):
+        sc.gz[layer] = gz[layer].data_ptr()
+        if layer == 0:
+            chunks = lib.vss_first_weight_grad_chunks_bf16x6(band, wd[1], wd[0])
+        else:
+            chunks = lib.vss_weight_grad_chunks_bf16x6(band, wd[layer + 1], wd[layer])
+        wpart = torch.empty((chunks, wd[layer + 1], wd[layer]), **f32)
+        bchunks = blocks if layer == n - 2 else lib.vss_linear_tanh_backward_chunks_bf16x6(band, wd[layer + 2], wd[layer + 1])
+        bpart = torch.empty((bchunks, wd[layer + 1]), **f32)
+        pt.wgrad[layer], pt.bias[layer] = wpart.data_ptr(), bpart.data_ptr()
+        defer.append((wpart, ws[layer].grad))
+        defer.append((bpart, bs[layer].grad))
+    c = float(clip_coef)
+    rin = N.VssMlpRows(obs=obs.data_ptr(), action=N.ptr(act), logprob_old=N.ptr(logp), adv=N.ptr(adv),
+                       adv_part=N.ptr(adv_part), adv_nparts=adv_part.shape[0] if adv_part is not None else 0,
+                       adv_count=float(adv_count), logstd=N.ptr(logstd), returns=N.ptr(ret),
+                       values_old=N.ptr(val) if clip_vloss else None, clip_coef=c, clip_lo=1 - c, clip_hi=1 + c,
+                       vf_coef=float(vf_coef), clip_vloss=int(bool(clip_vloss)))
+    N.check(lib.vss_mlp_train_banded_bf16x6(N.stream_of(obs.device), ctypes.byref(net), ctypes.byref(rin), rows, rows_pad,
+                                            band, ctypes.byref(sc), ctypes.byref(pt)), "vss_mlp_train_banded_bf16x6")
+    if scratch is not None:
+        scratch.update(h=hs, gz=gz, widths=wd, band=band)
+    del ws_c, bs_c
+    return stats
+
+
+
 def linear_tanh_mixed(x: torch.Tensor, w: torch.Tensor, b: torch.Tensor, planes: torch.Tensor | None = None) -> torch.Tensor:
     rows, k = x.shape
     n = w.shape[0]
```

New measurement: 1.698 billion env-steps/s, median of 5. About the same (+0.1%).
